# JakeKurtz/MC-Path-Tracer

Hardware: AMD Instinct MI355X
Metric: Mray/s (extend+shade) at 1080p x256spp depth5; fraction of HBM roofline (higher is better)
Workload: dtype f32

## Files before the change

### include/mcpt.h

```cpp
#ifndef MCPT_H
#define MCPT_H
#include <stdint.h>

#ifdef __cplusplus
extern "C" {
#endif

#define MCPT_ABI_VERSION 1

enum {
    MCPT_OK = 0,
    MCPT_E_INVALID = -1,
    MCPT_E_HIP = -2,
    MCPT_E_IO = -3,
    MCPT_E_NOMEM = -4,
    MCPT_E_NODEVICE = -5
};

typedef struct mcpt_config {
    uint64_t seed;
    int32_t spp;
    int32_t max_depth;
    int32_t rr_depth;
    int32_t tile_w;
// ... 32 lines not shown
typedef struct mcpt_camera {
    float inv_view_proj[16];
    float inv_view[16];
    float lens_radius;
    float focal;
} mcpt_camera;

typedef struct mcpt_camera_params {
    float position[3];
    float yaw_deg, pitch_deg;
    float fovy_rad, aspect, znear, zfar;
    float lens_radius, focal;
} mcpt_camera_params;

typedef struct mcpt_stage_stats {
    uint64_t extend_rays;
    uint64_t shadow_rays;
    uint64_t vis_rays;
    uint64_t iterations;
    uint64_t live_paths;
    float ms_total;
    float ms_shade;
    float ms_extend;
    float ms_shadow;
    uint64_t ext_nodes;
    uint64_t ext_tests;
    uint64_t ext_hits;
    uint64_t any_nodes, any_tests, any_hits;
} mcpt_stage_stats;

enum { MCPT_STAGE_LOGIC = 0, MCPT_STAGE_GENERATE = 1, MCPT_STAGE_MATERIAL = 2,
       MCPT_STAGE_EXTEND = 3, MCPT_STAGE_SHADOW = 4 };

typedef struct mcpt_path_view {
    uint32_t film_w, film_h;
    uint32_t *flags, *samples;
    int32_t *hit_tri;
    float *ray_o, *ray_d, *beta, *nee0, *nee1;
    uint8_t *vis;
    float *Ld;
    float *light_o, *light_d, *bvis_o, *bvis_d;
    uint8_t *queued;
} mcpt_path_view;

typedef struct mcpt_soa_view {
    const float *ray_o;
    const float *ray_d;
    float *hit_pos_t;
    float *hit_nrm_mat;
    int32_t *hit_tri;
    uint8_t *visible;
    uint32_t *steps;
    mcpt_path_view *paths;
} mcpt_soa_view;

typedef struct mcpt_ctx mcpt_ctx;
typedef struct mcpt_scene mcpt_scene;

int mcpt_create(int device, const mcpt_config *cfg, mcpt_ctx **out);
void mcpt_destroy(mcpt_ctx *ctx);
const char *mcpt_last_error(const mcpt_ctx *ctx);
int mcpt_scene_upload(mcpt_ctx *ctx, const mcpt_scene_desc *desc);
#define MCPT_GPU_BVH_LBVH 0
#define MCPT_GPU_BVH_PLOC 1
int mcpt_scene_upload_gpu_bvh(mcpt_ctx *ctx, const mcpt_scene_desc *desc);
int mcpt_set_gpu_bvh_builder(mcpt_ctx *ctx, int32_t builder);
#define MCPT_GEOM_REFIT   0
#define MCPT_GEOM_REBUILD 1
int mcpt_scene_update_geometry(mcpt_ctx *ctx, int32_t ntri,
                               const float *v0, const float *v1, const float *v2,
                               const float *n0, const float *n1, const float *n2,
                               int32_t mode);
int mcpt_scene_update_geometry_device(mcpt_ctx *ctx, int32_t ntri, const void *d_v0, const void *d_v1,
                                      const void *d_v2, const void *d_n0, const void *d_n1, const void *d_n2,
                                      int32_t mode);
int mcpt_debug_geometry_update_ms(const mcpt_ctx *ctx, float *out8);
int mcpt_camera_set(mcpt_ctx *ctx, const mcpt_camera *cam);
int mcpt_film_resize(mcpt_ctx *ctx, uint32_t w, uint32_t h, uint32_t tile_w, uint32_t tile_h);
int mcpt_film_clear(mcpt_ctx *ctx);
int mcpt_set_path_slots(mcpt_ctx *ctx, uint32_t slots);
int mcpt_set_trace_partitions(mcpt_ctx *ctx, uint32_t nparts);
int mcpt_set_work_counters(mcpt_ctx *ctx, int32_t on);
int mcpt_set_skip_discarded(mcpt_ctx *ctx, int32_t on);
int mcpt_set_tiles(mcpt_ctx *ctx, const uint32_t *tile_xy, uint32_t ntiles);
int mcpt_set_compact_paths(mcpt_ctx *ctx, int32_t on);
int mcpt_wavefront_step(mcpt_ctx *ctx, uint32_t tile_x, uint32_t tile_y, mcpt_stage_stats *st);
int mcpt_iterate(mcpt_ctx *ctx, uint32_t iterations, mcpt_stage_stats *st);
int mcpt_render(mcpt_ctx *ctx, mcpt_stage_stats *st);
int mcpt_stage_run(mcpt_ctx *ctx, int stage, const mcpt_soa_view *in, mcpt_soa_view *out, uint32_t n);
int mcpt_film_read(mcpt_ctx *ctx, float *Ld_rgb, uint32_t *samples);
int mcpt_film_read_device(mcpt_ctx *ctx, void *d_Ld_rgb, void *d_samples);
int mcpt_film_pack_tiles(mcpt_ctx *ctx, void *d_out, uint32_t *npix);
int mcpt_film_unpack_tiles(mcpt_ctx *ctx, const void *d_in, const uint32_t *tile_xy, uint32_t ntiles);
int mcpt_film_tonemap_rgba8(mcpt_ctx *ctx, float exposure, uint8_t *out);
int mcpt_film_size(const mcpt_ctx *ctx, uint32_t *w, uint32_t *h);
int mcpt_gather(mcpt_ctx *const *ctxs, int32_t n, int32_t root);
int mcpt_film_write_png(mcpt_ctx *ctx, float exposure, const char *path);
int mcpt_film_write_pfm(mcpt_ctx *ctx, const char *path);
int mcpt_image_write_png(const char *path, uint32_t w, uint32_t h, const uint8_t *rgba8);
int mcpt_image_write_pfm(const char *path, uint32_t w, uint32_t h, const float *rgb);
int mcpt_guides_render(mcpt_ctx *ctx, uint32_t nsamples);
int mcpt_guides_read(mcpt_ctx *ctx, float *albedo_rgb, float *normal_xyz, float *depth, uint32_t *count);
typedef struct mcpt_denoise_params {
    int32_t passes;
    float sigma_color;
    float sigma_normal, sigma_albedo, sigma_depth;
} mcpt_denoise_params;
int mcpt_denoise_default_params(mcpt_denoise_params *p);
int mcpt_denoise_run(mcpt_ctx *ctx, uint32_t w, uint32_t h, const float *rgb, const uint32_t *samples,
                     const float *albedo, const float *normal, const float *depth, const mcpt_denoise_params *p,
                     float *out_rgb);
int mcpt_film_denoise(mcpt_ctx *ctx, const mcpt_denoise_params *p);
int mcpt_denoised_read(mcpt_ctx *ctx, float *rgb);
int mcpt_denoised_read_device(mcpt_ctx *ctx, void *d_rgb);
int mcpt_denoised_tonemap_rgba8(mcpt_ctx *ctx, float exposure, uint8_t *out);
int mcpt_denoised_write_png(mcpt_ctx *ctx, float exposure, const char *path);
int mcpt_debug_denoise_ms(const mcpt_ctx *ctx, float *out10);
typedef struct mcpt_denoise_guided_params {
    int32_t passes;
    float sigma_lum;
    float lum_eps;
    float sigma_color;
    float sigma_normal, sigma_albedo, sigma_depth;
} mcpt_denoise_guided_params;
int mcpt_denoise_guided_default_params(mcpt_denoise_guided_params *p);
int mcpt_denoise_guided_run(mcpt_ctx *ctx, uint32_t w, uint32_t h, const float *rgb, const uint32_t *samples,
                            const float *variance, const float *albedo, const float *normal, const float *depth,
                            const mcpt_denoise_guided_params *p, float *out_rgb, float *out_variance);
int mcpt_film_denoise_guided(mcpt_ctx *ctx, const mcpt_denoise_guided_params *p);
int mcpt_denoised_variance_read(mcpt_ctx *ctx, float *var);
int mcpt_set_sample_budget(mcpt_ctx *ctx, const uint32_t *budget);
int mcpt_sample_budget_read(mcpt_ctx *ctx, uint32_t *out);
int mcpt_set_spp(mcpt_ctx *ctx, int32_t spp);
int mcpt_film_error(mcpt_ctx *ctx);
int mcpt_film_error_read(mcpt_ctx *ctx, float *out4);
int mcpt_error_run(mcpt_ctx *ctx, uint32_t w, uint32_t h, uint32_t slots, const float *Ld_slots,
                   const uint32_t *samples_slots, float *out4);
int mcpt_debug_film_read_slot(mcpt_ctx *ctx, uint32_t slot, float *Ld_rgb, uint32_t *samples);
typedef struct mcpt_sample_budget_params {
    float target_rel_err;
    float lum_floor;
    uint32_t min_spp, max_spp;
} mcpt_sample_budget_params;
int mcpt_sample_budget_default_params(mcpt_sample_budget_params *p);
int mcpt_budget_from_error(mcpt_ctx *ctx, const mcpt_sample_budget_params *p, uint64_t *out3);
int64_t mcpt_debug_adaptive_bytes(const mcpt_ctx *ctx);
int mcpt_debug_adaptive_ms(const mcpt_ctx *ctx, float *out2);
int mcpt_set_seed(mcpt_ctx *ctx, uint64_t seed);
int mcpt_camera_view_proj(const mcpt_camera *cam, float *out16);
typedef struct mcpt_temporal_params {
    float pos_tol;
    float nrm_tol;
    float max_history;
    float alpha_min;
} mcpt_temporal_params;
int mcpt_temporal_default_params(mcpt_temporal_params *p);
int mcpt_film_temporal(mcpt_ctx *ctx, const mcpt_temporal_params *p);
int mcpt_temporal_reset(mcpt_ctx *ctx);
int mcpt_temporal_read(mcpt_ctx *ctx, float *rgb, float *nsamples, float *variance, float *position);
int mcpt_temporal_denoise(mcpt_ctx *ctx, const mcpt_denoise_guided_params *p);
int mcpt_temporal_run(mcpt_ctx *ctx, uint32_t w, uint32_t h, const float *rgb, const uint32_t *samples,
                      const float *variance, const float *position, const float *normal, const float *depth,
                      const float *hcol, const float *hpos, const float *hnrm, const float *vp_prev16,
                      const mcpt_temporal_params *p, float *out_col, float *out_vl, float *out_hcol, float *out_hpos,
                      float *out_hnrm);
int64_t mcpt_debug_temporal_bytes(const mcpt_ctx *ctx);
int mcpt_debug_temporal_ms(const mcpt_ctx *ctx, float *out1);
typedef struct mcpt_variance_params {
    int32_t radius;
    float sigma_normal, sigma_albedo, sigma_depth;
    float min_neff;
} mcpt_variance_params;
int mcpt_variance_default_params(mcpt_variance_params *p);
int mcpt_variance_run(mcpt_ctx *ctx, uint32_t w, uint32_t h, const float *rgb, const uint32_t *samples,
                      const float *variance, const float *albedo, const float *normal, const float *depth,
                      const mcpt_variance_params *p, float *out_variance);
int mcpt_set_variance_fill(mcpt_ctx *ctx, const mcpt_variance_params *p);
int mcpt_debug_variance_ms(const mcpt_ctx *ctx, float *out1);
int mcpt_set_material_emission(mcpt_ctx *ctx, int32_t nmat, const float *rgb);
int mcpt_material_emission_read(mcpt_ctx *ctx, float *rgb, int32_t *nmat);
int mcpt_set_emitter_sampling(mcpt_ctx *ctx, int32_t on);
int mcpt_emitter_table_read(mcpt_ctx *ctx, float *cdf, float *pick, uint32_t *tri_id, int32_t *n);
int mcpt_debug_emitter_stats(const mcpt_ctx *ctx, double *out4);
int mcpt_sync(mcpt_ctx *ctx);
int mcpt_device_name(mcpt_ctx *ctx, char *buf, int32_t len);
int mcpt_debug_queue_rays(mcpt_ctx *ctx, int which, float *ray_o, float *ray_d, uint32_t *n_inout);
float mcpt_debug_last_stage_ms(const mcpt_ctx *ctx);
int mcpt_debug_tiny_lds_stack(mcpt_ctx *ctx, int32_t on);
float mcpt_debug_last_build_ms(const mcpt_ctx *ctx);
float mcpt_debug_last_env_build_ms(const mcpt_ctx *ctx);
int mcpt_debug_env_tables(mcpt_ctx *ctx, float *marginal_y, float *conds_y, float *pdf, int32_t *flags);
int mcpt_debug_node_layout(const mcpt_ctx *ctx);
typedef struct mcpt_bvh_info {
    int32_t npairs;
    int32_t root_ref;
    int32_t depth;
    int32_t width;
    int32_t layout;
    int32_t ntri;
    int32_t tri_f4;
    int32_t gpu_built;
    int32_t rounds;
    float root_mn[3], root_mx[3];
    float cull_p;
} mcpt_bvh_info;
int mcpt_debug_bvh_read(mcpt_ctx *ctx, float *nodes, float *tris, mcpt_bvh_info *info);
int mcpt_debug_occ_stats(const mcpt_ctx *ctx, uint64_t *resolved, int32_t *enabled);
int mcpt_debug_occ_complete_stats(const mcpt_ctx *ctx, double *out4);
int mcpt_debug_ray_counts(const mcpt_ctx *ctx, uint64_t *out);
int mcpt_debug_primary_stats(const mcpt_ctx *ctx, double *out4);
int mcpt_debug_discard_stats(const mcpt_ctx *ctx, uint64_t *out4);
int mcpt_debug_trace_profile(mcpt_ctx *ctx, uint64_t *out12, int reset);
int mcpt_debug_shade_sections(mcpt_ctx *ctx, uint64_t *out, int n, int reset);
int mcpt_debug_quot(mcpt_ctx *ctx, const float *a, const float *b, uint32_t n, float *out);
int mcpt_debug_hbm_copy(mcpt_ctx *ctx, uint64_t bytes, uint32_t iters, double *gbps);

mcpt_scene *mcpt_scene_new(void);
void mcpt_scene_free(mcpt_scene *s);
int mcpt_scene_load_glb(mcpt_scene *s, const char *path, const float *xform16);
int mcpt_scene_add_mesh(mcpt_scene *s, int32_t ntri, const float *v0, const float *v1, const float *v2,
                        const float *n0, const float *n1, const float *n2, const float *base_rgb);
int mcpt_scene_set_material_emission(mcpt_scene *s, int32_t mat, const float *rgb);
int mcpt_scene_get_emission(const mcpt_scene *s, const float **rgb, int32_t *nmat);
int mcpt_scene_set_env_hdr(mcpt_scene *s, const char *path, int32_t mode);
#define MCPT_ENV_DEVICE_TABLES 1
int mcpt_scene_set_env_hdr_ex(mcpt_scene *s, const char *path, int32_t mode, uint32_t flags);
int mcpt_scene_set_env_color(mcpt_scene *s, const float *rgb, float ls);
int mcpt_scene_add_dir_light(mcpt_scene *s, const float *dir, const float *rgb, float ls);
int mcpt_scene_transform(mcpt_scene *s, const float *xform16);
int mcpt_scene_make_proxy(mcpt_scene *s, int32_t config_id, const char *asset_dir);
int mcpt_scene_build(mcpt_scene *s, int32_t max_prims_in_node);
#define MCPT_BVH_REFERENCE 0
#define MCPT_BVH_SAH3 1
typedef struct mcpt_bvh_params {
    int32_t builder;
    int32_t max_prims;
    int32_t buckets;
    float trav_cost;
    float isect_cost;
} mcpt_bvh_params;
int mcpt_scene_build_ex(mcpt_scene *s, const mcpt_bvh_params *p);
int mcpt_scene_get_desc(const mcpt_scene *s, mcpt_scene_desc *out);
int mcpt_scene_bvh_depth(const mcpt_scene *s);
int mcpt_camera_make(const mcpt_camera_params *p, mcpt_camera *out);

#ifdef __cplusplus
}
#endif
#endif
```

### include/mcpt.hpp

```cpp
#ifndef MCPT_HPP
#define MCPT_HPP

#include <algorithm>
#include <array>
#include <atomic>
#include <cmath>
#include <cstdint>
#include <cstring>
#include <memory>
#include <stdexcept>
#include <string>
#include <utility>
#include <vector>

#include "mcpt.h"

namespace mcpt {

class Error : public std::runtime_error {
public:
    Error(int code, const std::string& what) : std::runtime_error(what), code_(code) {}
    int code() const { return code_; }

private:
// ... 363 lines not shown
    float get_exposure() const { return exposure; }
    void get_size(uint32_t& w, uint32_t& h) const { w = width; h = height; }
    void get_tile_size(uint32_t& w, uint32_t& h) const { w = tile_width; h = tile_height; }
    uint32_t get_id() const { return id; }
    void clear() {
        tile_id = 0;
        tile_x_pos = 0;
        tile_y_pos = 0;
        ++clears_;
        notify();
    }
    void update_tile_position() {
        tile_id = (tile_id + 1) % nmb_tiles;
        tile_x_pos = tile_id % nmb_tile_cols;
        tile_y_pos = tile_id / nmb_tile_cols;
    }
    uint32_t get_tile_x_pos() const { return tile_x_pos; }
    uint32_t get_tile_y_pos() const { return tile_y_pos; }
    uint32_t get_nmb_tiles() const { return nmb_tiles; }
    const std::vector<uint8_t>& get_image() const { return image; }
    uint64_t clear_count() const { return clears_; }

private:
    friend class PathTracer;
    void update_tile_info() {
        nmb_tile_cols = tile_width ? (width + tile_width - 1) / tile_width : 0;
        nmb_tile_rows = tile_height ? (height + tile_height - 1) / tile_height : 0;
        nmb_tiles = std::max(1u, nmb_tile_cols * nmb_tile_rows);
        nmb_tile_cols = std::max(1u, nmb_tile_cols);
    }
    uint32_t id = detail::gen_id();
    uint32_t width = 1, height = 1, tile_width = 0, tile_height = 0;
    uint32_t tile_id = 0, nmb_tiles = 1, nmb_tile_cols = 1, nmb_tile_rows = 1, tile_x_pos = 0, tile_y_pos = 0;
    float exposure = 1.f;
    uint64_t clears_ = 0;
    std::vector<uint8_t> image;
};

inline mcpt_config default_config() {
    mcpt_config c{0x5EED2026ull, 250, 5, 3, 256, 256, 0};
    return c;
}

class PathTracer {
public:
    explicit PathTracer(int device = 0, mcpt_config cfg = default_config()) : cfg_(cfg) {
        cfg.flags |= MCPT_FLAG_NO_AUTO_CLEAR;
        detail::check(mcpt_create(device, &cfg, &ctx_), nullptr, "PathTracer");
    }
    ~PathTracer() { mcpt_destroy(ctx_); }
    PathTracer(const PathTracer&) = delete;
    PathTracer& operator=(const PathTracer&) = delete;

    const std::vector<uint8_t>& render_image(const std::shared_ptr<Scene>& scene, const std::shared_ptr<Camera>& camera,
                                             const std::shared_ptr<Film>& film) {
        sync(*scene, *camera, *film);
        detail::check(mcpt_wavefront_step(ctx_, film->tile_x_pos, film->tile_y_pos, &stats_), ctx_, "render_image");
        if (display_) tonemap(*film);
        film->update_tile_position();
        return film->image;
    }
    const mcpt_stage_stats& render_iterations(const std::shared_ptr<Scene>& scene, const std::shared_ptr<Camera>& camera,
                                              const std::shared_ptr<Film>& film, uint32_t iterations) {
        sync(*scene, *camera, *film);
        detail::check(mcpt_iterate(ctx_, iterations, &stats_), ctx_, "render_iterations");
        if (display_) tonemap(*film);
        return stats_;
    }
    const mcpt_stage_stats& render_frame(const std::shared_ptr<Scene>& scene, const std::shared_ptr<Camera>& camera,
                                         const std::shared_ptr<Film>& film) {
        sync(*scene, *camera, *film);
        detail::check(mcpt_render(ctx_, &stats_), ctx_, "render_frame");
        if (display_) tonemap(*film);
        return stats_;
    }

    void clear_queues() {}
    void set_samples(int) {}
    int get_samples() { return 0; }

    void set_path_slots(uint32_t slots) {
        detail::check(mcpt_set_path_slots(ctx_, slots), ctx_, "set_path_slots");
    }
    void set_display(bool on) { display_ = on; }
    const mcpt_stage_stats& last_stats() const { return stats_; }
    const mcpt_config& config() const { return cfg_; }
    mcpt_ctx* handle() const { return ctx_; }
    std::string device_name() const {
        char buf[256] = {0};
        detail::check(mcpt_device_name(ctx_, buf, (int32_t)sizeof(buf)), ctx_, "device_name");
        return buf;
    }
    void read_film(std::vector<float>& Ld, std::vector<uint32_t>& samples) {
        uint32_t w = 0, h = 0;
        detail::check(mcpt_film_size(ctx_, &w, &h), ctx_, "read_film");
        Ld.resize((size_t)w * h * 3);
        samples.resize((size_t)w * h);
        detail::check(mcpt_film_read(ctx_, Ld.data(), samples.data()), ctx_, "read_film");
    }
    void write_png(const std::shared_ptr<Film>& film, const std::string& path) {
        detail::check(mcpt_film_write_png(ctx_, film->get_exposure(), path.c_str()), ctx_, "write_png");
    }
    void write_pfm(const std::string& path) {
        detail::check(mcpt_film_write_pfm(ctx_, path.c_str()), ctx_, "write_pfm");
    }
    void denoise(uint32_t guide_samples = 4, const mcpt_denoise_params* params = nullptr) {
        if (guide_samples) detail::check(mcpt_guides_render(ctx_, guide_samples), ctx_, "guides");
        detail::check(mcpt_film_denoise(ctx_, params), ctx_, "denoise");
    }
    void denoise_guided(uint32_t guide_samples = 4, const mcpt_denoise_guided_params* params = nullptr) {
        if (guide_samples) detail::check(mcpt_guides_render(ctx_, guide_samples), ctx_, "guides");
        detail::check(mcpt_film_denoise_guided(ctx_, params), ctx_, "denoise_guided");
    }
    void set_variance_fill(bool on = true, const mcpt_variance_params* params = nullptr) {
        mcpt_variance_params p;
        if (on && !params) detail::check(mcpt_variance_default_params(&p), ctx_, "set_variance_fill");
        detail::check(mcpt_set_variance_fill(ctx_, on ? (params ? params : &p) : nullptr), ctx_, "set_variance_fill");
    }
    void denoised_variance(std::vector<float>& var) {
        uint32_t w = 0, h = 0;
        detail::check(mcpt_film_size(ctx_, &w, &h), ctx_, "denoised_variance");
        var.resize((size_t)w * h);
        detail::check(mcpt_denoised_variance_read(ctx_, var.data()), ctx_, "denoised_variance");
    }
    void denoised(std::vector<float>& rgb) {
        uint32_t w = 0, h = 0;
        detail::check(mcpt_film_size(ctx_, &w, &h), ctx_, "denoised");
        rgb.resize((size_t)w * h * 3);
        detail::check(mcpt_denoised_read(ctx_, rgb.data()), ctx_, "denoised");
    }
    void write_denoised_png(const std::shared_ptr<Film>& film, const std::string& path) {
        detail::check(mcpt_denoised_write_png(ctx_, film->get_exposure(), path.c_str()), ctx_, "write_denoised_png");
    }
    void set_seed(uint64_t seed) {
        detail::check(mcpt_set_seed(ctx_, seed), ctx_, "set_seed");
        cfg_.seed = seed;
    }
    void temporal_accumulate(uint32_t guide_samples = 4, const mcpt_temporal_params* params = nullptr) {
        if (guide_samples) detail::check(mcpt_guides_render(ctx_, guide_samples), ctx_, "guides");
        detail::check(mcpt_film_temporal(ctx_, params), ctx_, "temporal_accumulate");
    }
    void temporal(std::vector<float>& rgb, std::vector<float>& nsamples, std::vector<float>& variance) {
        uint32_t w = 0, h = 0;
        detail::check(mcpt_film_size(ctx_, &w, &h), ctx_, "temporal");
        rgb.resize((size_t)w * h * 3);
        nsamples.resize((size_t)w * h);
        variance.resize((size_t)w * h);
        detail::check(mcpt_temporal_read(ctx_, rgb.data(), nsamples.data(), variance.data(), nullptr), ctx_, "temporal");
    }
    void temporal_denoise(const mcpt_denoise_guided_params* params = nullptr) {
        detail::check(mcpt_temporal_denoise(ctx_, params), ctx_, "temporal_denoise");
    }
    void temporal_reset() { detail::check(mcpt_temporal_reset(ctx_), ctx_, "temporal_reset"); }
    void update_geometry(const std::vector<float>& v0, const std::vector<float>& v1, const std::vector<float>& v2,
                         const std::vector<float>* n0 = nullptr, const std::vector<float>* n1 = nullptr,
                         const std::vector<float>* n2 = nullptr, int32_t mode = MCPT_GEOM_REFIT) {
        if (v0.size() % 3 || v1.size() != v0.size() || v2.size() != v0.size() || (n0 && n0->size() != v0.size()) ||
            (n1 && n1->size() != v0.size()) || (n2 && n2->size() != v0.size()))
            throw Error(MCPT_E_INVALID, "update_geometry: arrays of 3 floats per triangle, all of one size");
        detail::check(mcpt_scene_update_geometry(ctx_, (int32_t)(v0.size() / 3), v0.data(), v1.data(), v2.data(),
                                                 n0 ? n0->data() : nullptr, n1 ? n1->data() : nullptr,
                                                 n2 ? n2->data() : nullptr, mode),
                      ctx_, "update_geometry");
    }
    std::array<float, 8> geometry_update_ms() const {
        std::array<float, 8> ms{};
// ... 138 lines not shown
```

### mc-path-tracer_amd/csrc/kernels.hip

```cpp
#include <hip/hip_runtime.h>
#include <stdint.h>
#include <stdlib.h>
#include <string.h>
#include <algorithm>

#include "device/mcpt_core.hpp"
#include "device/scene_dev.hpp"
#include "kernels.hpp"

using namespace mcpt;

namespace mcpt_dev {

template <int NQ>
__device__ inline void block_push(const bool (&want)[NQ], uint32_t* const (&counters)[NQ], uint32_t (&slot)[NQ],
                                  uint32_t (&total)[NQ]) {
    __shared__ uint32_t s_wave[NQ][kBlock / 64];
    __shared__ uint32_t s_base[NQ];
    __shared__ uint32_t s_tot[NQ];
    const int lane = threadIdx.x & 63, wave = threadIdx.x >> 6;
    uint32_t prefix[NQ];
#pragma unroll
    for (int q = 0; q < NQ; q++) {
        uint64_t m = __ballot(want[q]);
        prefix[q] = __builtin_amdgcn_mbcnt_hi((uint32_t)(m >> 32), __builtin_amdgcn_mbcnt_lo((uint32_t)m, 0u));
        if (lane == 0) s_wave[q][wave] = (uint32_t)__popcll(m);
    }
    __syncthreads();
    if (threadIdx.x < NQ) {
        const int q = threadIdx.x;
        uint32_t tot = 0;
        for (int w = 0; w < kBlock / 64; w++) { uint32_t c = s_wave[q][w]; s_wave[q][w] = tot; tot += c; }
        s_base[q] = tot ? atomicAdd(counters[q], tot) : 0u;
        s_tot[q] = tot;
    }
    __syncthreads();
#pragma unroll
    for (int q = 0; q < NQ; q++) {
        slot[q] = s_base[q] + s_wave[q][wave] + prefix[q];
        total[q] = s_tot[q];
    }
}

template <class T>
__device__ inline const T& kernarg_fresh() {
    typedef const __attribute__((address_space(4))) T KT;
    KT* p = (KT*)__builtin_amdgcn_kernarg_segment_ptr();
    __asm__ volatile("" : "+s"(p));
    return *(const T*)p;
}


#ifndef MCPT_NT
#define MCPT_NT 3
#endif
template <class T>
__device__ inline void st_q(T* p, T v) {
    if constexpr (MCPT_NT & 8) __builtin_nontemporal_store(v, p);
    else *p = v;
}
typedef float f4v_t __attribute__((ext_vector_type(4)));
typedef uint32_t u4v_t __attribute__((ext_vector_type(4)));
template <class T>
__device__ inline T ld_s(const T* p) {
    if constexpr (MCPT_NT & 1) return __builtin_nontemporal_load(p);
    else return *p;
}
__device__ inline float4 ld_s(const float4* p) {
    if constexpr (MCPT_NT & 1) {
        const f4v_t v = __builtin_nontemporal_load(reinterpret_cast<const f4v_t*>(p));
        return make_float4(v.x, v.y, v.z, v.w);
    } else {
        return *p;
    }
}
__device__ inline uint4 ld_s(const uint4* p) {
    if constexpr (MCPT_NT & 1) {
        const u4v_t v = __builtin_nontemporal_load(reinterpret_cast<const u4v_t*>(p));
        return make_uint4(v.x, v.y, v.z, v.w);
    } else {
        return *p;
    }
}
template <class T>
__device__ inline void st_s(T* p, T v) {
    if constexpr (MCPT_NT & 2) __builtin_nontemporal_store(v, p);
    else *p = v;
}
// ... 1 lines not shown
    if constexpr (MCPT_NT & 2) __builtin_nontemporal_store(f4v_t{v.x, v.y, v.z, v.w}, reinterpret_cast<f4v_t*>(p));
    else *p = v;
}
__device__ inline void st_s(uint4* p, uint4 v) {
    if constexpr (MCPT_NT & 2) __builtin_nontemporal_store(u4v_t{v.x, v.y, v.z, v.w}, reinterpret_cast<u4v_t*>(p));
    else *p = v;
}

enum : int { SD_WAVES = 0, SD_VALID, SD_LOGIC, SD_NEE, SD_GEN, SD_CONT, SD_BG, SD_N };
#ifdef MCPT_DIAG_SHADE
__device__ unsigned long long g_shade_diag[2 * SD_N];
#define SHADE_DIAG(k, cond)                                                      \
    do {                                                                         \
        const uint64_t m_ = __ballot(cond);                                      \
        if ((threadIdx.x & 63) == 0 && m_) {                                     \
            atomicAdd(&g_shade_diag[2 * (k)], 1ull);                             \
            atomicAdd(&g_shade_diag[2 * (k) + 1], (unsigned long long)__popcll(m_)); \
        }                                                                        \
    } while (0)
#else
#define SHADE_DIAG(k, cond) \
    do {                    \
    } while (0)
#endif
int shade_sections(unsigned long long* out, int n, int reset) {
#ifdef MCPT_DIAG_SHADE
    unsigned long long h[2 * SD_N];
    if (hipMemcpyFromSymbol(h, HIP_SYMBOL(g_shade_diag), sizeof(h)) != hipSuccess) return -1;
    for (int i = 0; i < n && i < 2 * SD_N; i++) out[i] = h[i];
    if (reset) {
        memset(h, 0, sizeof(h));
        if (hipMemcpyToSymbol(HIP_SYMBOL(g_shade_diag), h, sizeof(h)) != hipSuccess) return -1;
    }
    return 2 * SD_N;
#else
    for (int i = 0; i < n; i++) out[i] = 0;
    (void)reset;
    return 0;
#endif
}

__device__ inline V3 light_L(const DevScene& sc, int id, V3 wi) {
    if (id == 0) return env_L(sc.env, wi);
    const float* p = sc.dirs + 7 * (id - 1);
    return v3(p[3], p[4], p[5]) * p[6];
}
template <bool FIXED>
__device__ inline void light_L_pdf(const DevScene& sc, int id, V3 wi, V3& L, float& pdf) {
    if (id == 0) {
        env_L_pdf<FIXED>(sc.env, wi, L, pdf);
    } else {
        const float* p = sc.dirs + 7 * (id - 1);
        L = v3(p[3], p[4], p[5]) * p[6];
        pdf = 1.f;
    }
}
__device__ inline float light_pdf(const DevScene& sc, int id, V3 wi) {
    if (id == 0) return env_pdf(sc.env, wi);
    return 1.f;
}

__device__ inline bool slab(float mnx, float mny, float mnz, float mxx, float mxy, float mxz, V3 o, V3 inv,
                            int nx, int ny, int nz, float& t0, float& t1) {
    float bx0 = nx ? mxx : mnx, bx1 = nx ? mnx : mxx;
    float by0 = ny ? mxy : mny, by1 = ny ? mny : mxy;
    float bz0 = nz ? mxz : mnz, bz1 = nz ? mnz : mxz;
    float tmin = (bx0 - o.x) * inv.x;
    float tmax = (bx1 - o.x) * inv.x;
    float tymin = (by0 - o.y) * inv.y;
    float tymax = (by1 - o.y) * inv.y;
    float tzmin = (bz0 - o.z) * inv.z;
    float tzmax = (bz1 - o.z) * inv.z;
    bool miss = (tmin > tymax) || (tymin > tmax);
    float a = (tymin > tmin) ? tymin : tmin;
    float b = (tymax < tmax) ? tymax : tmax;
    miss = miss || (a > tzmax) || (tzmin > b);
    t0 = (tzmin > a) ? tzmin : a;
    t1 = (tzmax < b) ? tzmax : b;
    return !miss;
}
constexpr float K_INF_F = __builtin_huge_valf();

__device__ inline float cull_iota(const DevScene& sc, V3 d, V3 inv) {
    const float ax = __builtin_fabsf(inv.x), ay = __builtin_fabsf(inv.y), az = __builtin_fabsf(inv.z);
    if (!(ax < K_INF_F && ay < K_INF_F && az < K_INF_F)) return -K_INF_F;
    const float n2 = d.x * d.x + d.y * d.y + d.z * d.z;
    if (!sc.cull_ok || !(n2 <= kCullNormMax)) return -3.4028235e38f;
    const float io = __builtin_fmaxf(__builtin_fmaxf(ax, ay), az) * kCullSlackF;
    return io * sc.cull_p <= 1.f ? io : -io;
}
__device__ inline bool keep_box(float t0, float t1, float m, float cut, float& key) {
    key = t0 - __builtin_fabsf(m);
    return !(m >= 0.f && __builtin_fmaf(t1, kCullBehindF, m) < 0.f) && !(key > cut);
}

typedef float f2v __attribute__((ext_vector_type(2)));
__device__ inline void pair_slab(float4 qx, float4 qy, float4 qz, V3 o, V3 inv, float& t0a, float& t1a, float& t0b,
                                 float& t1b) {
    const f2v ox = {o.x, o.x}, oy = {o.y, o.y}, oz = {o.z, o.z};
    const f2v ix = {inv.x, inv.x}, iy = {inv.y, inv.y}, iz = {inv.z, inv.z};
    const f2v ax = (f2v{qx.x, qx.y} - ox) * ix, bx = (f2v{qx.z, qx.w} - ox) * ix;
    const f2v ay = (f2v{qy.x, qy.y} - oy) * iy, by = (f2v{qy.z, qy.w} - oy) * iy;
    const f2v az = (f2v{qz.x, qz.y} - oz) * iz, bz = (f2v{qz.z, qz.w} - oz) * iz;
    t0a = __builtin_fmaxf(__builtin_fmaxf(__builtin_fminf(ax.x, bx.x), __builtin_fminf(ay.x, by.x)),
                          __builtin_fminf(az.x, bz.x));
    t1a = __builtin_fminf(__builtin_fminf(__builtin_fmaxf(ax.x, bx.x), __builtin_fmaxf(ay.x, by.x)),
                          __builtin_fmaxf(az.x, bz.x));
    t0b = __builtin_fmaxf(__builtin_fmaxf(__builtin_fminf(ax.y, bx.y), __builtin_fminf(ay.y, by.y)),
                          __builtin_fminf(az.y, bz.y));
    t1b = __builtin_fminf(__builtin_fminf(__builtin_fmaxf(ax.y, bx.y), __builtin_fmaxf(ay.y, by.y)),
                          __builtin_fmaxf(az.y, bz.y));
}

__device__ inline void quad_axis(const float4& mn, const float4& mx, float o, float inv, float (&lo)[4],
                                 float (&hi)[4], bool first) {
    const f2v oo = {o, o}, ii = {inv, inv};
    const f2v a0 = (f2v{mn.x, mn.y} - oo) * ii, a1 = (f2v{mn.z, mn.w} - oo) * ii;
    const f2v b0 = (f2v{mx.x, mx.y} - oo) * ii, b1 = (f2v{mx.z, mx.w} - oo) * ii;
    const float l[4] = {__builtin_fminf(a0.x, b0.x), __builtin_fminf(a0.y, b0.y), __builtin_fminf(a1.x, b1.x),
                        __builtin_fminf(a1.y, b1.y)};
    const float h[4] = {__builtin_fmaxf(a0.x, b0.x), __builtin_fmaxf(a0.y, b0.y), __builtin_fmaxf(a1.x, b1.x),
                        __builtin_fmaxf(a1.y, b1.y)};
#pragma unroll
    for (int k = 0; k < 4; k++) {
        lo[k] = first ? l[k] : __builtin_fmaxf(lo[k], l[k]);
        hi[k] = first ? h[k] : __builtin_fminf(hi[k], h[k]);
    }
}

__device__ inline f2v pk_slab(f2v q, f2v p) {
    f2v r;
    __asm__("v_pk_add_f32 %0, %1, %2 op_sel_hi:[1,0] neg_lo:[0,1] neg_hi:[0,1]\n\t"
            "v_pk_mul_f32 %0, %0, %2 op_sel:[0,1] op_sel_hi:[1,1]"
            : "=&v"(r)
            : "v"(q), "v"(p));
    return r;
}
__device__ inline void box_t(float ax, float bx, float ay, float by, float az, float bz, float& t0, float& t1) {
    float m0, m1, m2, n0, n1, n2;
    __asm__("v_min_f32 %2, %8, %9\n\t"
            "v_min_f32 %3, %10, %11\n\t"
            "v_min_f32 %4, %12, %13\n\t"
            "v_max_f32 %5, %8, %9\n\t"
            "v_max_f32 %6, %10, %11\n\t"
            "v_max_f32 %7, %12, %13\n\t"
            "v_max3_f32 %0, %2, %3, %4\n\t"
            "v_min3_f32 %1, %5, %6, %7"
            : "=v"(t0), "=v"(t1), "=&v"(m0), "=&v"(m1), "=&v"(m2), "=&v"(n0), "=&v"(n1), "=&v"(n2)
            : "v"(ax), "v"(bx), "v"(ay), "v"(by), "v"(az), "v"(bz));
}
__device__ inline void pair_slab2(float4 qx, float4 qy, float4 qz, f2v px, f2v py, f2v pz, float& t0a, float& t1a,
                                  float& t0b, float& t1b) {
    const f2v ax = pk_slab(f2v{qx.x, qx.y}, px), bx = pk_slab(f2v{qx.z, qx.w}, px);
    const f2v ay = pk_slab(f2v{qy.x, qy.y}, py), by = pk_slab(f2v{qy.z, qy.w}, py);
    const f2v az = pk_slab(f2v{qz.x, qz.y}, pz), bz = pk_slab(f2v{qz.z, qz.w}, pz);
    box_t(ax.x, bx.x, ay.x, by.x, az.x, bz.x, t0a, t1a);
    box_t(ax.y, bx.y, ay.y, by.y, az.y, bz.y, t0b, t1b);
}
__device__ inline float vmin(float a, float b) {
    float r;
    __asm__("v_min_f32 %0, %1, %2" : "=v"(r) : "v"(a), "v"(b));
    return r;
}
__device__ inline float vmax(float a, float b) {
    float r;
    __asm__("v_max_f32 %0, %1, %2" : "=v"(r) : "v"(a), "v"(b));
    return r;
}
__device__ inline void quad_axis2(const float4& mn, const float4& mx, f2v p, float (&lo)[4], float (&hi)[4], bool first) {
    const f2v a0 = pk_slab(f2v{mn.x, mn.y}, p), a1 = pk_slab(f2v{mn.z, mn.w}, p);
    const f2v b0 = pk_slab(f2v{mx.x, mx.y}, p), b1 = pk_slab(f2v{mx.z, mx.w}, p);
    const float l[4] = {vmin(a0.x, b0.x), vmin(a0.y, b0.y), vmin(a1.x, b1.x), vmin(a1.y, b1.y)};
    const float h[4] = {vmax(a0.x, b0.x), vmax(a0.y, b0.y), vmax(a1.x, b1.x), vmax(a1.y, b1.y)};
#pragma unroll
    for (int k = 0; k < 4; k++) {
        lo[k] = first ? l[k] : vmax(lo[k], l[k]);
        hi[k] = first ? h[k] : vmin(hi[k], h[k]);
    }
}

__device__ inline bool ray_misses_scene(const DevScene& sc, V3 o, V3 d) {
    if (!(d.x == d.x && d.y == d.y && d.z == d.z) || (d.x == 0.f && d.y == 0.f && d.z == 0.f)) return true;
    if (o.x >= sc.root_mn[0] && o.x <= sc.root_mx[0] && o.y >= sc.root_mn[1] && o.y <= sc.root_mx[1] &&
        o.z >= sc.root_mn[2] && o.z <= sc.root_mx[2])
        return false;
    const V3 inv = v3(1.f / d.x, 1.f / d.y, 1.f / d.z);
    const float m = sc.root_w * cull_iota(sc, d, inv);
    float t0, t1, key;
    return !(slab(sc.root_mn[0], sc.root_mn[1], sc.root_mn[2], sc.root_mx[0], sc.root_mx[1], sc.root_mx[2], o, inv,
                  inv.x < 0.f, inv.y < 0.f, inv.z < 0.f, t0, t1) &&
             keep_box(t0, t1, m, K_INF_F, key));
}

__device__ inline bool occ_test(V3 o, V3 d, V3 inv, float io, float4 bmn, float4 bmx, float4 r2, float4 r3) {
    const float ax = (bmn.x - o.x) * inv.x, bx = (bmx.x - o.x) * inv.x;
    const float ay = (bmn.y - o.y) * inv.y, by = (bmx.y - o.y) * inv.y;
    const float az = (bmn.z - o.z) * inv.z, bz = (bmx.z - o.z) * inv.z;
    const float t0 = __builtin_fmaxf(__builtin_fmaxf(__builtin_fminf(ax, bx), __builtin_fminf(ay, by)),
                                     __builtin_fminf(az, bz));
    const float t1 = __builtin_fminf(__builtin_fminf(__builtin_fmaxf(ax, bx), __builtin_fmaxf(ay, by)),
                                     __builtin_fmaxf(az, bz));
    float key;
    if (!(t0 <= t1) || !keep_box(t0, t1, bmn.w * io, K_INF_F, key)) return false;
    float th;
    return tri_test_t(o, d, v3(bmx.w, r2.x, r2.y), v3(r2.z, r2.w, r3.x), v3(r3.y, r3.z, r3.w), th) && !(th < 0.f) &&
           th < K_HUGE;
}
struct OccEnt { uint32_t w[kOccWays]; };
__device__ inline OccEnt occ_entry(const DevScene& sc, uint32_t cell) {
    typedef uint32_t uwv_t __attribute__((ext_vector_type(kOccWays)));
    const uwv_t* e = reinterpret_cast<const uwv_t*>(sc.occ) + cell;
    uwv_t v;
    if constexpr (MCPT_NT & 16) v = __builtin_nontemporal_load(e);
    else v = *e;
    OccEnt r;
#pragma unroll
    for (uint32_t k = 0; k < kOccWays; k++) r.w[k] = v[k];
    return r;
}
enum : int { kOccOpen = 0, kOccHit = 1, kOccMaybe = 2 };
__device__ inline int occ_hit1(const DevScene& sc, V3 o, V3 d, OccEnt e, bool& done) {
    done = sc.occ_dir != nullptr;
    bool any = false;
#pragma unroll
    for (uint32_t k = 0; k < kOccWays; k++) done = done && mcpt::occ_word_done(e.w[k]);
#pragma unroll
    for (uint32_t k = 0; k < kOccWays; k++) {
        if (done) e.w[k] &= mcpt::kOccDoneIndex;
        any = any || e.w[k] < sc.ntri;
    }
    if (!(any || done)) return kOccOpen;
    const V3 inv = v3(1.f / d.x, 1.f / d.y, 1.f / d.z);
    const bool fin = __builtin_fabsf(inv.x) < K_INF_F && __builtin_fabsf(inv.y) < K_INF_F && __builtin_fabsf(inv.z) < K_INF_F;
    const float io = cull_iota(sc, d, inv);
#pragma unroll
    for (uint32_t k = 0; k < kOccWays; k += 2) {
        const bool v0 = e.w[k] < sc.ntri, v1 = e.w[k + 1] < sc.ntri;
        if (kOccWays > 2 && !(v0 || v1)) continue;
        const float4* p0 = sc.occ_rec + kOccRecF4 * (size_t)(v0 ? e.w[k] : 0u);
        const float4* p1 = sc.occ_rec + kOccRecF4 * (size_t)(v1 ? e.w[k + 1] : 0u);
        const float4 bn0 = p0[0], bx0 = p0[1], r20 = p0[2], r30 = p0[3];
        const float4 bn1 = p1[0], bx1 = p1[1], r21 = p1[2], r31 = p1[3];
        if (!fin) return kOccOpen;
        if ((v0 && occ_test(o, d, inv, io, bn0, bx0, r20, r30)) || (v1 && occ_test(o, d, inv, io, bn1, bx1, r21, r31)))
            return kOccHit;
    }
    return done && fin && io > 0.f ? kOccMaybe : kOccOpen;
}
__device__ inline void occ_member2(const DevScene& sc, V3 ol, V3 dl, uint32_t kl, V3 ob, V3 db, uint32_t kb, bool& m_l,
                                   bool& m_b) {
    const mcpt::OccGrid g{{sc.root_mn[0], sc.root_mn[1], sc.root_mn[2]}, {sc.occ_cell[0], sc.occ_cell[1], sc.occ_cell[2]},
                          sc.occ_g, sc.occ_b, sc.occ_dir};
    const mcpt::Beam bl = mcpt::occ_key_beam(g, (kl >> 15) & 31u, (kl >> 20) & 31u, kl >> 25, kl & 0x7fffu);
    const mcpt::Beam bb = mcpt::occ_key_beam(g, (kb >> 15) & 31u, (kb >> 20) & 31u, kb >> 25, kb & 0x7fffu);
    m_l = mcpt::beam_contains(bl, ol, dl);
    m_b = mcpt::beam_contains(bb, ob, db);
}

struct MatOut {
    bool want_ext, want_l, want_b, trivial_ext, vis_ray, need_cb;
    bool skip_ext;
    bool doomed_inplace;
    uint32_t trivial_any;
    OccEnt el, eb;
    uint32_t kl, kb;
    V3 n, wo, wi_b;
    int matid, light_id;
    uint32_t flags;
    float rrz;
};

template <bool FIXED, bool SAMP = false>
__device__ inline MatOut material(const ShadeArgs& a, uint32_t pid, uint32_t pix, uint32_t sidx, uint32_t len,
                                 V3 beta_store, int32_t htri, float4* stage, bool occ_on, bool no_cont, bool& want_e) {
    const DevScene& sc = a.scene;
    MatOut mo{};
#pragma unroll
    for (uint32_t k = 0; k < kOccWays; k++) mo.el.w[k] = mo.eb.w[k] = kOccEmpty;
    MCPT_MARK("m_hit");
    const Rng r{rng_key(a.seed, pix, sidx), len};
    const V3 ro = xyz(ld_s(a.p.ray_o + pid)), rdir = xyz(ld_s(a.p.ray_d + pid));
    V3 pos, n;
    int mat;
    float t_hit;
    hit_record(sc, ro, rdir, htri, pos, n, mat, t_hit);
    const V3 wo = -rdir;
    const Mat m = load_mat(sc.mats + 8 * mat);
    uint32_t nf = 0;
    V3 rr;
    if (no_cont) {
        rr = v3(0.f, 0.f, 0.f);
        st_s(a.p.beta + pid, f4(beta_store, 0.f));
        mo.skip_ext = true;
    } else {
        MCPT_MARK("m_cont");
        V3 wi_s = brdf_sample_wi<FIXED>(m, n, wo, r, SL_CONT_E0, r(SL_CONT_LOBE) < 0.5f);
        float pdf_s;
        V3 f_s;
        brdf_f_pdf(m, n, wi_s, wo, f_s, pdf_s);
        if ((f_s.x == 0.f && f_s.y == 0.f && f_s.z == 0.f) || pdf_s == 0.f) nf |= F_FZERO;
        rr = f_s / pdf_s;
        const V3 new_o = pos + n * 0.001f;
        st_s(a.p.beta + pid, f4(beta_store, rr.x));
        bool doomed = false;
        if (FIXED || !a.skip) {
            doomed = len + 1u > (uint32_t)a.max_depth;
            if (!doomed && len + 1u > (uint32_t)a.rr_depth) {
                const Rng r1{r.key, len + 1u};
                float q;
                doomed = rr_terminates(r1, FIXED ? (beta_store * rr).y : beta_store.y, q);
            }
        }
        if (doomed && a.skip) {
            mo.skip_ext = true;
        } else {
            st_s(a.p.ray_o + pid, f4(new_o, 0.f));
            st_s(a.p.ray_d + pid, f4(wi_s, 0.f));
            mo.want_ext = true;
            if (ray_misses_scene(sc, new_o, wi_s)) {
                a.p.hit_tri[pid] = -1;
                mo.want_ext = false;
                mo.trivial_ext = true;
                mo.doomed_inplace = doomed;
            }
        }
    }
    MCPT_MARK("m_light");
    int l_id = (int)(r(SL_LIGHT) * (float)(sc.nlights - 0) + (float)0);
    const int light_id = (l_id == sc.nlights) ? 0 : l_id;
    const bool delta = light_id > 0;
    const float sel = FIXED ? 1.f / (float)sc.nlights : 1.f;
    {
        V3 ldir, Li_l;
        float pdfl_x;
        const float4* lt = sc.env.ltab[FIXED ? 1 : 0];
        if (light_id == 0 && lt) {
            int cx, cy;
            env_cell<FIXED>(sc.env, r, cx, cy);
            const float4 t0 = lt[(int64_t)cy * (sc.env.w + 1) + cx + 1];
            const float2 rs = sc.env.lrow[FIXED ? 1 : 0][cy], cs = sc.env.lcol[FIXED ? 1 : 0][cx + 1];
            ldir = v3(cs.y * rs.x, rs.y, cs.x * rs.x);
            pdfl_x = t0.w;
            Li_l = xyz(t0);
        } else {
            if (light_id == 0) ldir = env_dir<FIXED>(sc.env, r);
            else ldir = ld3(sc.dirs + 7 * (light_id - 1), 0);
            light_L_pdf<FIXED>(sc, light_id, ldir, Li_l, pdfl_x);
        }
        V3 f_l;
        float pdf_bl;
        brdf_f_pdf(m, n, ldir, wo, f_l, pdf_bl);
        if (FIXED) pdfl_x = pdfl_x * sel;
        float pdfb_y = !delta ? pdf_bl : (FIXED ? 0.f : 1.f);
        float wL = power_heuristic(pdfl_x, pdfb_y);
        V3 cL = ((f_l * Li_l) * wL) / pdfl_x;
        if (wL > 0.f && pdfl_x > 0.f) nf |= F_CONDL;
        st_s(a.p.nee0 + pid, f4(cL, rr.y));
        const V3 so_l = pos + n * 0.01f;
        if (ray_misses_scene(sc, so_l, ldir)) {
            a.p.vis[2 * pid] = 1;
            mo.trivial_any++;
        } else {
            stage[0 * kBlock + threadIdx.x] = f4(so_l, __uint_as_float(2 * pid));
            stage[1 * kBlock + threadIdx.x] = f4(ldir, 0.f);
            mo.want_l = true;
            if (occ_on) mo.el = occ_entry(sc, occ_index(sc, so_l, ldir, &mo.kl));
        }
    }
    if constexpr (SAMP) {
        MCPT_MARK("m_emit");
        int k = upper_bound(a.emit_cdf, a.emit_n, r(SL_EMIT_PICK));
        k = k < a.emit_n - 1 ? k : a.emit_n - 1;
        const uint2 ent = a.emit_ent[k];
        const float4* tp = sc.tri + (size_t)kTriF4 * ent.x;
        const float4 w0 = tp[0], w1 = tp[1], w2 = tp[2];
        const V3 ev0 = v3(w0.x, w0.y, w0.z), e1 = v3(w0.w, w1.x, w1.y), e2 = v3(w1.z, w1.w, w2.x);
        const float u1 = r(SL_EMIT_U), u2 = r(SL_EMIT_V), su = __builtin_sqrtf(u1);
        const V3 pe = (ev0 + e1 * (su * (1.f - u2))) + e2 * (su * u2);
        const V3 so_e = pos + n * 0.01f;
        const V3 dv = pe - so_e;
        const float d2 = dot(dv, dv), dist = __builtin_sqrtf(d2);
        const V3 edir = dv / dist;
        const V3 c = cross(e1, e2);
        const float area = 0.5f * __builtin_sqrtf(dot(c, c));
        const float cosl = __builtin_fabsf(dot(normalize(c), edir));
        const float pdf_e = ((__uint_as_float(ent.y) / area) * d2) / cosl;
        V3 f_e;
        float pdf_be;
        brdf_f_pdf(m, n, edir, wo, f_e, pdf_be);
        const int mat_e = __float_as_int(sc.tri_sh[3 * (size_t)ent.x + 2].y);
        V3 cE = (f_e * ld3f4(a.emis + mat_e)) / pdf_e;
        const bool ok = dist > 0.f && cosl > 0.f && pdf_e > 0.f && pdf_e < K_INF_F && __builtin_fabsf(cE.x) < K_INF_F &&
                        __builtin_fabsf(cE.y) < K_INF_F && __builtin_fabsf(cE.z) < K_INF_F;
        if (ok) {
            stage[4 * kBlock + threadIdx.x] = f4(so_e, __uint_as_float(a.emit_vis0 + pid));
            stage[5 * kBlock + threadIdx.x] = f4(edir, dist * 0.999f);
            want_e = true;
        } else {
            cE = v3(0.f, 0.f, 0.f);
            a.p.vis[a.emit_vis0 + pid] = 0;
        }
        st_s(a.nee2 + pid, f4(cE, 0.f));
    }
    MCPT_MARK("m_bsdir");
    if (!delta) {
        const V3 wi_b = brdf_sample_wi<FIXED>(m, n, wo, r, SL_MAT_E0, r(SL_MAT_LOBE) < 0.5f);
// ... 294 lines not shown
            const uint32_t qi = shard * a.ext_cap + slot[1];
            st_s(a.mat_rec + qi, make_uint4(pid, pix, cont_sidx | (no_cont ? kRecNoCont : 0u) | (cont_len << kRecLenShift),
                                            (uint32_t)cont_htri));
            st_s(a.mat_beta + qi, f4(beta_store, 0.f));
        }
    }
    uint32_t n_ext = ((gen_ext || gen_trivial || gen_prim) ? 1u : 0u) + (dd ? 1u : 0u);
    for (int off = 32; off > 0; off >>= 1) n_ext += __shfl_xor(n_ext, off);
    if (lane == 0 && n_ext) atomicAdd(sc_ctr + C_EXT_RAYS, n_ext);
    if (a.skip) {
        const uint32_t n_dd = (uint32_t)__popcll(__ballot(dd)), n_ddv = (uint32_t)__popcll(__ballot(dd_vis));
        if (lane == 0 && n_dd) {
            atomicAdd(sc_ctr + C_ANY_RAYS, n_dd + n_ddv);
            if (n_ddv) atomicAdd(sc_ctr + C_VIS, n_ddv);
            atomicAdd(sc_ctr + C_SKIP_EXT, n_dd);
            atomicAdd(sc_ctr + C_SKIP_ANY, n_dd + n_ddv);
            atomicAdd(sc_ctr + C_SKIP_MAT, n_dd);
        }
    }
    if (a.prim_cnt) {
        const uint32_t n_prim = (uint32_t)__popcll(__ballot(prim_res));
        if (lane == 0 && n_prim) atomicAdd(sc_ctr + C_PRIM_RAYS, n_prim);
    }
    MCPT_MARK("background");
    if (bg) {
        const int nbg = FIXED ? 1 : sc.nlights;
        V3 film = bg_film;
        for (int i = 0; i < nbg; i++) film = film + env_L(sc.env, bg_dir) * v3(1.f, 1.f, 1.f);
        if (__float_as_uint(film.x) != __float_as_uint(bg_film.x) || __float_as_uint(film.y) != __float_as_uint(bg_film.y) ||
            __float_as_uint(film.z) != __float_as_uint(bg_film.z))
            a.p.Ld[pid] = f4(film, 0.f);
    }
    if constexpr (EMIT) {
        MCPT_MARK("emission");
        if (em) {
            const int mat = __float_as_int(sc.tri_sh[3 * cont_htri + 2].y);
            const V3 film = bg_film + ld3f4(a.emis + mat) * beta_store;
            if (em_dirty || __float_as_uint(film.x) != __float_as_uint(bg_film.x) ||
                __float_as_uint(film.y) != __float_as_uint(bg_film.y) || __float_as_uint(film.z) != __float_as_uint(bg_film.z))
                a.p.Ld[pid] = f4(film, 0.f);
        }
    }
    MCPT_MARK("done");
    if (a.blk_done && __syncthreads_and(finished ? 1 : 0) && threadIdx.x == 0) a.blk_done[v.done] = 1;
    MCPT_MARK("end");
}

template <bool FIXED, bool MAP, bool EMIT, bool SAMP = false>
__global__ __launch_bounds__(kBlock) MCPT_SHADE_ATTR void k_shade(ShadeArgs a) {
    if (a.cnt->idle) return;
    __shared__ uint64_t s_live[kBlock / 64];
    const uint32_t G = gridDim.x, nvb = a.shade_vblocks;
    const uint32_t mine = (nvb - blockIdx.x + G - 1) / G;
    const uint32_t k = threadIdx.x;
    bool live = false;
    __shared__ VBlk s_vb[kBlock];
    if (k < mine) {
        const VBlk v = vblock_of(a, (int)(blockIdx.x + k * G));
        live = !a.blk_done || a.blk_done[v.done] == 0;
        s_vb[k] = v;
    }
    const uint64_t m = __ballot(live);
    if ((threadIdx.x & 63) == 0) s_live[threadIdx.x >> 6] = m;
    __syncthreads();
    for (uint32_t j = 0; j < mine; j++) {
        if (!((s_live[j >> 6] >> (j & 63)) & 1ull)) continue;
        shade_vblock<FIXED, MAP, EMIT, SAMP>(kernarg_fresh<ShadeArgs>(), (int)(blockIdx.x + j * G), s_vb[j]);
    }
}

template <bool FIXED, bool SAMP = false>
__global__ __launch_bounds__(kBlock) MCPT_MAT_ATTR void k_material(ShadeArgs a_kernarg) {
    (void)a_kernarg;
    const ShadeArgs& a = kernarg_fresh<ShadeArgs>();
    if (a.cnt->idle) return;
    const uint32_t shard = blockIdx.x % kShards, w_in = blockIdx.x / kShards, bps = gridDim.x / kShards;
    uint32_t* sc_ctr = a.cnt->shard[shard];
    const uint32_t n = sc_ctr[C_MAT];
    const int lane = threadIdx.x & 63;
    uint32_t n_ext = 0, n_any = 0, n_vis = 0, n_occ = 0, occ_try = 0, n_skip = 0, n_inpl = 0, n_dvis = 0, n_docc = 0;
    uint32_t n_emit = 0;
    (void)n_emit;
    const bool occ_on = a.scene.occ && a.scene.occ_gate[0] == 0 && a.scene.occ_gate[2] != 0;
    __shared__ float4 s_any[SAMP ? 6 : 4][kBlock];
    for (uint32_t base = w_in * kBlock; base < n; base += bps * kBlock) {
        const ShadeArgs& a = kernarg_fresh<ShadeArgs>();
        const uint32_t i = base + threadIdx.x;
        MatOut mo{};
        bool want_e = false;
        uint32_t mpid = 0;
        bool occ_l = false, occ_b = false, try_l = false, try_b = false;
        bool done_l = false, done_b = false, clr_l = false, clr_b = false;
        if (i < n) {
            const uint4 q = ld_s(a.mat_rec + shard * a.ext_cap + i);
            const float4 b4 = ld_s(a.mat_beta + shard * a.ext_cap + i);
            mpid = q.x;
            mo = material<FIXED, SAMP>(a, mpid, q.y, q.z & (kRecNoCont - 1u), q.z >> kRecLenShift, xyz(b4), (int32_t)q.w,
                                 &s_any[0][0], occ_on, (q.z & kRecNoCont) != 0u, want_e);
            MCPT_MARK("m_occ");
            if (occ_on) {
                try_l = mo.want_l;
                try_b = mo.want_b;
                const V3 ol = xyz(s_any[0][threadIdx.x]), dl = xyz(s_any[1][threadIdx.x]);
                const V3 ob = xyz(s_any[2][threadIdx.x]), db = xyz(s_any[3][threadIdx.x]);
                if (mo.want_l) {
                    const int r = occ_hit1(a.scene, ol, dl, mo.el, done_l);
                    occ_l = r == kOccHit;
                    clr_l = r == kOccMaybe;
                }
                if (mo.want_b) {
                    const int r = occ_hit1(a.scene, ob, db, mo.eb, done_b);
                    occ_b = r == kOccHit;
                    clr_b = r == kOccMaybe;
                }
                if (clr_l || clr_b) {
                    bool m_l, m_b;
                    occ_member2(a.scene, ol, dl, mo.kl, ob, db, mo.kb, m_l, m_b);
                    clr_l = clr_l && m_l;
                    clr_b = clr_b && m_b;
                }
                if (clr_l) {
                    a.p.vis[2 * mpid] = 1;
                    mo.want_l = false;
                    mo.trivial_any++;
                }
                if (clr_b) {
                    a.p.vis[2 * mpid + 1] = 1;
                    mo.want_b = false;
                    mo.trivial_any++;
                }
                if (occ_l) {
                    a.p.vis[2 * mpid] = 0;
                    mo.want_l = false;
                    mo.trivial_any++;
                }
                if (occ_b) {
                    a.p.vis[2 * mpid + 1] = 0;
                    mo.want_b = false;
                    mo.need_cb = false;
                    mo.trivial_any++;
                }
            }
            MCPT_MARK("m_bterms");
            material_brdf_terms<FIXED>(a, mpid, mo);
        }
        MCPT_MARK("m_push");
        uint32_t slot[SAMP ? 4 : 3], total[SAMP ? 4 : 3];
        if constexpr (SAMP) {
            bool want[4] = {mo.want_ext, mo.want_l, mo.want_b, want_e};
            uint32_t* ctr[4] = {sc_ctr + C_EXT, sc_ctr + C_ANY, sc_ctr + C_ANY, sc_ctr + C_ANY};
            block_push<4>(want, ctr, slot, total);
        } else {
            bool want[3] = {mo.want_ext, mo.want_l, mo.want_b};
            uint32_t* ctr[3] = {sc_ctr + C_EXT, sc_ctr + C_ANY, sc_ctr + C_ANY};
            block_push<3>(want, ctr, slot, total);
        }
        if (mo.want_ext) st_q(a.ext_q + shard * a.ext_cap + slot[0], mpid);
        if (mo.want_l) {
            const uint32_t k = shard * a.any_cap + slot[1];
            if constexpr (MCPT_NT & 8) {
                st_s(a.p.sray_o + k, s_any[0][threadIdx.x]);
                st_s(a.p.sray_d + k, s_any[1][threadIdx.x]);
            } else {
                a.p.sray_o[k] = s_any[0][threadIdx.x];
                a.p.sray_d[k] = s_any[1][threadIdx.x];
            }
        }
        if (mo.want_b) {
            const uint32_t k = shard * a.any_cap + slot[2];
            if constexpr (MCPT_NT & 8) {
                st_s(a.p.sray_o + k, s_any[2][threadIdx.x]);
                st_s(a.p.sray_d + k, s_any[3][threadIdx.x]);
            } else {
                a.p.sray_o[k] = s_any[2][threadIdx.x];
                a.p.sray_d[k] = s_any[3][threadIdx.x];
            }
        }
        if constexpr (SAMP) {
            if (want_e) {
                const uint32_t k = shard * a.any_cap + slot[3];
                if constexpr (MCPT_NT & 8) {
                    st_s(a.p.sray_o + k, s_any[4][threadIdx.x]);
                    st_s(a.p.sray_d + k, s_any[5][threadIdx.x]);
                } else {
                    a.p.sray_o[k] = s_any[4][threadIdx.x];
                    a.p.sray_d[k] = s_any[5][threadIdx.x];
                }
            }
            n_emit += (uint32_t)__popcll(__ballot(want_e));
        }
        MCPT_MARK("m_count");
        n_occ += (uint32_t)(__popcll(__ballot(occ_l)) + __popcll(__ballot(occ_b)));
        occ_try += (uint32_t)(__popcll(__ballot(try_l)) + __popcll(__ballot(try_b)));
        n_dvis += (uint32_t)(__popcll(__ballot(clr_l)) + __popcll(__ballot(clr_b)));
        n_docc += (uint32_t)(__popcll(__ballot(occ_l && done_l)) + __popcll(__ballot(occ_b && done_b)));
        n_ext += (uint32_t)__popcll(__ballot(mo.want_ext || mo.trivial_ext || mo.skip_ext));
        n_skip += (uint32_t)__popcll(__ballot(mo.skip_ext));
        n_inpl += (uint32_t)__popcll(__ballot(mo.doomed_inplace));
        n_any += (uint32_t)(__popcll(__ballot(mo.want_l)) + __popcll(__ballot(mo.want_b)) +
                            __popcll(__ballot(mo.trivial_any >= 1u)) + __popcll(__ballot(mo.trivial_any >= 2u)));
        n_vis += (uint32_t)__popcll(__ballot(mo.vis_ray));
    }
    if (lane == 0) {
        if (n_ext) atomicAdd(sc_ctr + C_EXT_RAYS, n_ext);
        if (n_any) atomicAdd(sc_ctr + C_ANY_RAYS, n_any);
        if (n_vis) atomicAdd(sc_ctr + C_VIS, n_vis);
        if (n_occ) atomicAdd(sc_ctr + C_OCC, n_occ);
        if (occ_try) atomicAdd(sc_ctr + C_OCC_TRY, occ_try);
        if (n_dvis) atomicAdd(sc_ctr + C_OCC_DONE_VIS, n_dvis);
        if (n_docc) atomicAdd(sc_ctr + C_OCC_DONE_OCC, n_docc);
        if (n_skip) atomicAdd(sc_ctr + C_SKIP_EXT, n_skip);
        if (n_inpl) atomicAdd(sc_ctr + C_SKIP_INPLACE, n_inpl);
        if constexpr (SAMP)
            if (n_emit) atomicAdd(a.cnt->tot_emit + shard, (unsigned long long)n_emit);
    }
}

__device__ inline uint32_t wave_scan_incl(uint32_t x) {
    x += (uint32_t)__builtin_amdgcn_update_dpp(0, (int)x, 0x111, 0xf, 0xf, false);
    x += (uint32_t)__builtin_amdgcn_update_dpp(0, (int)x, 0x112, 0xf, 0xf, false);
    x += (uint32_t)__builtin_amdgcn_update_dpp(0, (int)x, 0x114, 0xf, 0xf, false);
    x += (uint32_t)__builtin_amdgcn_update_dpp(0, (int)x, 0x118, 0xf, 0xf, false);
    x += (uint32_t)__builtin_amdgcn_update_dpp(0, (int)x, 0x142, 0xa, 0xf, false);
    x += (uint32_t)__builtin_amdgcn_update_dpp(0, (int)x, 0x143, 0xc, 0xf, false);
    return x;
}

__device__ inline void wave_stats(uint32_t* stats, int lane, uint32_t nodes, uint32_t tests, uint32_t hits) {
    if (!stats) return;
    for (int off = 32; off > 0; off >>= 1) {
        nodes += __shfl_xor(nodes, off);
        tests += __shfl_xor(tests, off);
        hits += __shfl_xor(hits, off);
    }
    if (lane == 0) {
        uint32_t* st = stats + (blockIdx.x % kShards) * C_WORDS;
        atomicAdd(st + 0, nodes);
        atomicAdd(st + 1, tests);
        atomicAdd(st + 2, hits);
    }
}

#ifndef MCPT_NODE_STEPS
#define MCPT_NODE_STEPS 4
#endif
#ifndef MCPT_TRI_SHARE
#define MCPT_TRI_SHARE 0
#endif
constexpr int kShareMaxStack = 8;
constexpr int kNodeSteps = MCPT_NODE_STEPS;
#ifndef MCPT_GRAB_MAX
#define MCPT_GRAB_MAX 0
#endif
constexpr int kGrabMax = MCPT_GRAB_MAX;
#ifndef MCPT_ANY_FIRST
#define MCPT_ANY_FIRST 0
#endif
constexpr bool kAnyFirst = MCPT_ANY_FIRST != 0;
#ifndef MCPT_NODE_MIN_LANES2
#define MCPT_NODE_MIN_LANES2 32
#endif
#ifndef MCPT_NODE_MIN_LANES2_DEEP
#define MCPT_NODE_MIN_LANES2_DEEP 0
#endif
#ifndef MCPT_NODE_MIN_LANES4
#define MCPT_NODE_MIN_LANES4 24
#endif

#ifndef MCPT_TRACE_WPE
#define MCPT_TRACE_WPE 7
#endif
#ifndef MCPT_TRACE_WPE_DEEP
#define MCPT_TRACE_WPE_DEEP 7
#endif
#ifndef MCPT_TRACE_WPE4
#define MCPT_TRACE_WPE4 6
#endif
#define MCPT_TRACE_WPE_OF(kW, kS) \
    ((kW) == 4 ? MCPT_TRACE_WPE4 : ((kS) > ::mcpt_dev::kLdsStack ? MCPT_TRACE_WPE_DEEP : MCPT_TRACE_WPE))
#define MCPT_TRACE_ATTR \
    __attribute__((amdgpu_waves_per_eu(MCPT_TRACE_WPE_OF(kW, kLdsStack), MCPT_TRACE_WPE_OF(kW, kLdsStack))))
template <int kW, int kLdsStack, bool kCount>
__global__ __launch_bounds__(kTraceBlock) MCPT_TRACE_ATTR void k_trace(TraceArgs a) {
    if (a.idle && *a.idle) return;
    constexpr bool kShare = MCPT_TRI_SHARE != 0 && kLdsStack <= kShareMaxStack;
    __shared__ int2 stk[kLdsStack][kTraceBlock];
    __shared__ uint64_t s_key[kShare ? kTraceBlock : 1];
    const int lane = threadIdx.x;
    const uint32_t nsh = (uint32_t)a.nshards, nparts = a.nparts;
    uint32_t home = 0;
    if (nparts > 1) {
        uint32_t xcc;
        __asm__ volatile("s_getreg_b32 %0, hwreg(HW_REG_XCC_ID)" : "=s"(xcc));
        const uint32_t nd = a.ndies >= 1 && a.ndies <= nparts && nparts % a.ndies == 0 ? a.ndies : nparts;
        home = (xcc & 15u) % nd + nd * ((blockIdx.x / nd) % (nparts / nd));
// ... 418 lines not shown
                float t;
                bool done = false;
                const bool acc = tri_test_t(RAY_O, d, v3(w0.x, w0.y, w0.z), v3(w0.w, w1.x, w1.y), v3(w1.z, w1.w, w2.x), t);
                MCPT_MARK("t_tri2");
                if (acc && !(t < 0.f) &&
                    (best < 0.f ? t < -best
                          : (t < best ||
                             (t == best && tri >= 0 && __float_as_int(w2.y) < __float_as_int(sc.tri[kTriF4 * tri + 2].y))))) {
                    if (best < 0.f) {
                        tri = id;
                        done = true;
                    } else {
                        best = t;
                        tri = id;
                        cut = best * __builtin_fmaf(__builtin_fabsf(io), sc.cull_p, kCullSlackF);
                    }
                }
                if (done) {
                    leaf = kEnd;
                    ref = kEnd;
                } else if ((leaf & 0x07000000) != 0) {
                    leaf = leaf + 1 - (1 << 24);
                } else {
                    leaf = kEnd;
                }
            }
        }
        MCPT_MARK("t_finish");
        if constexpr (kCount) ph[PH_FINISH_TRIPS] += __ballot(act && ref == kEnd && leaf == kEnd) != 0 ? 1u : 0u;
        if (act && ref == kEnd && leaf == kEnd) finish();
        }
        MCPT_MARK("t_end");
    }
    MCPT_MARK("t_scan");
    {
        uint32_t g = 0;
        const bool cand = (uint32_t)lane < nparts && !((drained >> lane) & 1ull);
        if (cand) g = __hip_atomic_load(a.grab + lane * C_WORDS, __ATOMIC_RELAXED, __HIP_MEMORY_SCOPE_AGENT);
        const uint64_t open = __ballot(cand && g < s_tot[lane]);
        if (open == 0) break;
        const uint32_t rem = min(s_tot[lane] - g, (1u << 25) - 1u);
        uint32_t key = (open >> lane) & 1ull ? (rem << 6) | (63u - (uint32_t)lane) : 0u;
        for (int off = 32; off > 0; off >>= 1) key = max(key, (uint32_t)__shfl_xor((int)key, off));
        enter(63u - (__builtin_amdgcn_readfirstlane(key) & 63u));
    }
    }
#undef RAY_O
#undef RAY_INV
    if constexpr (kCount) {
        wave_stats(a.set[0].stats, lane, tot_n - tot_n1, tot_t - tot_t1, tot_h - tot_h1);
        wave_stats(a.set[1].stats, lane, tot_n1, tot_t1, tot_h1);
        if (a.phase && lane == 0) {
            uint32_t* pw = a.phase + (blockIdx.x % kShards) * C_WORDS;
#pragma unroll
            for (int k = 0; k < kPhaseWords; k++)
                if (ph[k]) atomicAdd(pw + k, ph[k]);
        }
    }
}

__global__ __launch_bounds__(kBlock) void k_primary(ShadeArgs a_kernarg) {
    (void)a_kernarg;
    const ShadeArgs& a = kernarg_fresh<ShadeArgs>();
    if (a.cnt->idle) return;
    const uint32_t shard = blockIdx.x % kShards, w_in = blockIdx.x / kShards, bps = gridDim.x / kShards;
    const uint32_t n = a.cnt->shard[shard][C_PRIM];
    const float4* rec = a.scene.occ_rec;
    for (uint32_t i = w_in * kBlock + threadIdx.x; i < n; i += bps * kBlock) {
        const uint2 q = a.prim_q[shard * a.ext_cap + i];
        const V3 o = ld3f4(a.p.ray_o + q.x), d = ld3f4(a.p.ray_d + q.x);
        const uint32_t nc = (uint32_t)a.prim_cnt[q.y] - 1u;
        const uint4* lp = reinterpret_cast<const uint4*>(a.prim_list + (size_t)kPrimLine * q.y);
        const V3 inv = v3(1.f / d.x, 1.f / d.y, 1.f / d.z);
        float best = K_HUGE;
        int32_t tri = -1;
        for (uint32_t j0 = 0; j0 < nc; j0 += 4) {
            const uint4 ids = lp[j0 >> 2];
            const uint32_t id4[4] = {ids.x, ids.y, ids.z, ids.w};
#pragma unroll
            for (int k = 0; k < 4; k++) {
                if (j0 + k >= nc) break;
                const float4* p = rec + kOccRecF4 * (size_t)id4[k];
                const float4 bmn = p[0], bmx = p[1], r2 = p[2], r3 = p[3];
                const float ax = (bmn.x - o.x) * inv.x, bx = (bmx.x - o.x) * inv.x;
                const float ay = (bmn.y - o.y) * inv.y, by = (bmx.y - o.y) * inv.y;
                const float az = (bmn.z - o.z) * inv.z, bz = (bmx.z - o.z) * inv.z;
                const float t0 = __builtin_fmaxf(__builtin_fmaxf(__builtin_fminf(ax, bx), __builtin_fminf(ay, by)),
                                                 __builtin_fminf(az, bz));
                const float t1 = __builtin_fminf(__builtin_fminf(__builtin_fmaxf(ax, bx), __builtin_fmaxf(ay, by)),
                                                 __builtin_fmaxf(az, bz));
                float t;
                if (t0 <= t1 && tri_test_t(o, d, v3(bmx.w, r2.x, r2.y), v3(r2.z, r2.w, r3.x), v3(r3.y, r3.z, r3.w), t) &&
                    !(t < 0.f) && t < best) {
                    best = t;
                    tri = (int32_t)id4[k];
                }
            }
        }
        a.p.hit_tri[q.x] = tri;
    }
}
void launch_primary(const ShadeArgs& a, const LaunchGeom& g, hipStream_t s) {
    if (a.prim_cnt) hipLaunchKernelGGL(k_primary, dim3(g.prim_blocks), dim3(kBlock), 0, s, a);
}

#ifndef MCPT_OCC_BACKOFF0
#define MCPT_OCC_BACKOFF0 15
#endif
__global__ void k_accumulate(CounterBlock* c, uint32_t nparts, uint32_t* occ_gate) {
    if (c->idle) return;
    const int t = threadIdx.x;
    uint32_t v[C_STATS + 6];
#pragma unroll
    for (int k = 0; k < C_STATS + 6; k++) {
        v[k] = c->shard[t][k];
        c->shard[t][k] = 0;
    }
    c->last_ext_shard[t] = v[C_EXT];
    __shared__ uint32_t s_part[kMaxParts];
    if (t < kMaxParts) s_part[t] = 0;
    __syncthreads();
    atomicAdd(&s_part[t % nparts], v[C_EXT] + v[C_ANY]);
    __syncthreads();
    uint32_t g = 0;
    if (t < kMaxParts) g = c->grab[t][0];
    const bool short_part = t < (int)nparts && g < s_part[t];
#pragma unroll
    for (int k = 0; k < C_STATS + 6; k++)
        for (int off = 32; off > 0; off >>= 1) v[k] += __shfl_xor(v[k], off);
    if (__ballot(short_part) != 0 && t == 0) c->trace_short += 1;
    if (t < kMaxParts) c->grab[t][0] = 0;
    uint32_t phw[kPhaseWords];
#pragma unroll
    for (int k = 0; k < kPhaseWords; k++) {
        phw[k] = c->shard[t][C_PH + k];
        c->shard[t][C_PH + k] = 0;
        for (int off = 32; off > 0; off >>= 1) phw[k] += __shfl_xor(phw[k], off);
    }
    uint32_t er = c->shard[t][C_EXT_RAYS], ar = c->shard[t][C_ANY_RAYS], oc = c->shard[t][C_OCC],
             ot = c->shard[t][C_OCC_TRY], pr = c->shard[t][C_PRIM_RAYS], dv = c->shard[t][C_OCC_DONE_VIS],
             dc = c->shard[t][C_OCC_DONE_OCC];
    const int skw[4] = {C_SKIP_EXT, C_SKIP_ANY, C_SKIP_MAT, C_SKIP_INPLACE};
    uint32_t sk[4];
#pragma unroll
    for (int k = 0; k < 4; k++) {
        sk[k] = c->shard[t][skw[k]];
        if (sk[k]) c->shard[t][skw[k]] = 0;
        for (int off = 32; off > 0; off >>= 1) sk[k] += __shfl_xor(sk[k], off);
    }
    c->shard[t][C_PRIM] = 0;
    c->shard[t][C_PRIM_RAYS] = 0;
    c->shard[t][C_EXT_RAYS] = 0;
    c->shard[t][C_ANY_RAYS] = 0;
    c->shard[t][C_MAT] = 0;
    c->shard[t][C_OCC] = 0;
    c->shard[t][C_OCC_TRY] = 0;
    if (dv) c->shard[t][C_OCC_DONE_VIS] = 0;
    if (dc) c->shard[t][C_OCC_DONE_OCC] = 0;
    for (int off = 32; off > 0; off >>= 1) {
        dv += __shfl_xor(dv, off);
        dc += __shfl_xor(dc, off);
        er += __shfl_xor(er, off);
        ar += __shfl_xor(ar, off);
        oc += __shfl_xor(oc, off);
        ot += __shfl_xor(ot, off);
        pr += __shfl_xor(pr, off);
    }
    if (t == 0) {
        c->tot_ext += er;
        c->tot_prim += pr;
        for (int k = 0; k < 4; k++) c->tot_skip[k] += sk[k];
        c->tot_any += ar;
        c->tot_occ += oc;
        c->tot_done[0] += dv;
        c->tot_done[1] += dc;
        if (occ_gate) {
            if (occ_gate[0]) {
                occ_gate[0]--;
            } else if (!occ_gate[2]) {
                if (v[C_ANY]) occ_gate[2] = 1;
            } else if (ot >= 4096u) {
                if (((unsigned long long)oc + dv) * kOccMinRate < ot) {
                    occ_gate[1] = occ_gate[1] ? min(2u * occ_gate[1] + 1u, 255u) : (uint32_t)MCPT_OCC_BACKOFF0;
                    occ_gate[0] = occ_gate[1];
                } else {
                    occ_gate[1] = 0;
                }
            }
        }
        c->tot_vis += v[C_VIS];
        c->tot_ext_q += v[C_EXT];
        c->tot_any_q += v[C_ANY];
        c->last_ext = v[C_EXT];
        c->last_live = er;
        if (er == 0) c->idle = 1;
        for (int k = 0; k < 6; k++) c->tot_stats[k] += v[C_STATS + k];
        for (int k = 0; k < kPhaseWords; k++) c->tot_phase[k] += phw[k];
    }
}
void launch_accumulate(CounterBlock* c, uint32_t nparts, uint32_t* occ_gate, hipStream_t s) {
    hipLaunchKernelGGL(k_accumulate, dim3(1), dim3(kShards), 0, s, c, std::min<uint32_t>(kMaxParts, std::max<uint32_t>(1, nparts)),
                       occ_gate);
}

static uint32_t env_u32(const char* name, int def, int lo, int hi) {
    const char* e = getenv(name);
    int v = e ? atoi(e) : def;
    return (uint32_t)std::min(hi, std::max(lo, v));
}
int launch_geometry(int dev, LaunchGeom& g) {
    int cus = 0, nx = 1, per_cu = 0, mat0 = 0, mat1 = 0, sh0 = 0;
    if (hipDeviceGetAttribute(&cus, hipDeviceAttributeMultiprocessorCount, dev) != hipSuccess) return -1;
    if (hipDeviceGetAttribute(&nx, hipDeviceAttributeNumberOfXccs, dev) != hipSuccess) nx = 1;
    int occ[2][2] = {};
    if (hipOccupancyMaxActiveBlocksPerMultiprocessor(&occ[0][0], k_trace<2, kLdsStack, false>, kTraceBlock, 0) != hipSuccess ||
        hipOccupancyMaxActiveBlocksPerMultiprocessor(&occ[0][1], k_trace<2, kLdsStackDeep, false>, kTraceBlock, 0) != hipSuccess ||
        hipOccupancyMaxActiveBlocksPerMultiprocessor(&occ[1][0], k_trace<4, kLdsStack, false>, kTraceBlock, 0) != hipSuccess ||
        hipOccupancyMaxActiveBlocksPerMultiprocessor(&occ[1][1], k_trace<4, kLdsStackDeep, false>, kTraceBlock, 0) != hipSuccess ||
        hipOccupancyMaxActiveBlocksPerMultiprocessor(&mat0, k_material<false>, kBlock, 0) != hipSuccess ||
        hipOccupancyMaxActiveBlocksPerMultiprocessor(&mat1, k_material<true>, kBlock, 0) != hipSuccess ||
        hipOccupancyMaxActiveBlocksPerMultiprocessor(&sh0, k_shade<false, false, false>, kBlock, 0) != hipSuccess)
        return -1;
    if (cus <= 0) cus = 256;
    per_cu = 32;
    if (const char* e = getenv("MCPT_TRACE_WAVES")) per_cu = atoi(e);
    if (per_cu <= 0) per_cu = 16;
    for (int w = 0; w < 2; w++)
        for (int k = 0; k < 2; k++) g.trace_waves[w][k] = (uint32_t)(cus * std::max(1, std::min(per_cu, occ[w][k])));
    g.ndies = (uint32_t)std::max(1, nx);
    g.trace_parts = env_u32("MCPT_TRACE_PARTS", std::min(kMaxParts, 2 * std::max(1, nx)), 1, kMaxParts);
    if (const char* e = getenv("MCPT_MAT_BLOCKS_PER_CU")) {
        const int m = atoi(e);
        if (m > 0) { mat0 = std::min(mat0, m); mat1 = std::min(mat1, m); }
    }
    g.mat_blocks[0] = (uint32_t)std::max(1, cus * std::max(1, mat0) / kShards) * (uint32_t)kShards;
    g.mat_blocks[1] = (uint32_t)std::max(1, cus * std::max(1, mat1) / kShards) * (uint32_t)kShards;
    {
        int ms0 = 0, ms1 = 0;
        if (hipOccupancyMaxActiveBlocksPerMultiprocessor(&ms0, k_material<false, true>, kBlock, 0) != hipSuccess ||
            hipOccupancyMaxActiveBlocksPerMultiprocessor(&ms1, k_material<true, true>, kBlock, 0) != hipSuccess)
            return -1;
        g.mat_blocks_samp[0] = (uint32_t)std::max(1, cus * std::max(1, ms0) / kShards) * (uint32_t)kShards;
        g.mat_blocks_samp[1] = (uint32_t)std::max(1, cus * std::max(1, ms1) / kShards) * (uint32_t)kShards;
    }
    int prim = 0;
    if (hipOccupancyMaxActiveBlocksPerMultiprocessor(&prim, k_primary, kBlock, 0) != hipSuccess) return -1;
    g.prim_blocks = (uint32_t)std::max(1, cus * std::max(1, prim) / kShards) * (uint32_t)kShards;
    g.shade_grid = (uint32_t)std::max(1, cus * std::max(1, sh0)) * env_u32("MCPT_SHADE_GRID", 16, 0, 1024);
    if (getenv("MCPT_SHADE_WGS")) g.shade_grid = env_u32("MCPT_SHADE_WGS", 0, 1, 1 << 30);
    g.refill_min = env_u32("MCPT_REFILL_MIN", 0, 0, 64);
    g.tri_min = env_u32("MCPT_TRI_MIN", 16, 0, 64);
    return 0;
}
static uint32_t shade_grid(uint32_t nblocks, const LaunchGeom& g) {
    uint32_t G = g.shade_grid ? std::min(nblocks, g.shade_grid) : nblocks;
    return std::max(G, (nblocks + kBlock - 1) / kBlock);
}
void launch_shade(const ShadeArgs& args, int nblocks, const LaunchGeom& g, bool fixed_mode, hipStream_t s) {
    ShadeArgs a = args;
    a.shade_vblocks = (uint32_t)nblocks;
    const uint32_t G = shade_grid((uint32_t)nblocks, g);
    if (a.nee2 && a.emis) {
        if (fixed_mode) {
            if (a.budget) hipLaunchKernelGGL((k_shade<true, true, true, true>), dim3(G), dim3(kBlock), 0, s, a);
            else hipLaunchKernelGGL((k_shade<true, false, true, true>), dim3(G), dim3(kBlock), 0, s, a);
            hipLaunchKernelGGL((k_material<true, true>), dim3(g.mat_blocks_samp[1]), dim3(kBlock), 0, s, a);
        } else {
            if (a.budget) hipLaunchKernelGGL((k_shade<false, true, true, true>), dim3(G), dim3(kBlock), 0, s, a);
            else hipLaunchKernelGGL((k_shade<false, false, true, true>), dim3(G), dim3(kBlock), 0, s, a);
            hipLaunchKernelGGL((k_material<false, true>), dim3(g.mat_blocks_samp[0]), dim3(kBlock), 0, s, a);
        }
        return;
    }
    if (fixed_mode) {
// ... 63 lines not shown
```

### mc-path-tracer_amd/csrc/kernels.hpp

```cpp
#pragma once
#include <hip/hip_runtime.h>
#include <stdint.h>

#include "device/adaptive.hpp"
#include "device/denoise.hpp"
#include "device/mcpt_core.hpp"
#include "device/occ_beam.hpp"
#include "device/temporal.hpp"
#include "device/variance.hpp"

namespace mcpt_dev {

constexpr int kBlock = 256;
constexpr int kTraceBlock = 64;
#ifndef MCPT_LDS_STACK
#define MCPT_LDS_STACK 8
#endif
constexpr int kLdsStack = MCPT_LDS_STACK;
#ifndef MCPT_LDS_STACK_DEEP
#define MCPT_LDS_STACK_DEEP 10
#endif
constexpr int kLdsStackDeep = MCPT_LDS_STACK_DEEP;
constexpr int kLdsStackTiny = 2;
#ifndef MCPT_DEEP_TREE
#define MCPT_DEEP_TREE 20
#endif
constexpr int kDeepTree = MCPT_DEEP_TREE;
constexpr int kMaxStack = 64;

enum : uint32_t {
    F_DEAD = 1u,
    F_LEN_SHIFT = 1,
    F_CONDL = 1u << 9,
    F_CONDB = 1u << 10,
    F_FZERO = 1u << 11,
    F_HASVIS = 1u << 12,
    F_SIDX_SHIFT = 13
};
constexpr uint32_t kMaxSpp = 1u << (32 - F_SIDX_SHIFT);
constexpr int kRecLenShift = 24;
static_assert(kMaxSpp <= (1u << kRecLenShift), "sample index and len share a record word");
constexpr uint32_t kRecNoCont = 1u << 23;
static_assert(kMaxSpp <= kRecNoCont && kRecNoCont < (1u << kRecLenShift), "the mark lies between sample index and len");

__host__ __device__ constexpr int shade_blocks_per_tile(int tile_px, int slots) {
    return (tile_px + kBlock - 1) / kBlock * slots;
}

#ifndef MCPT_TRI_F4
#define MCPT_TRI_F4 3
#endif
constexpr int kTriF4 = MCPT_TRI_F4;

struct DevScene {
    const float4* nodes;
    const float4* tri;
    const float4* tri_sh;
    float root_mn[3], root_mx[3];
    int root_ref;
    int depth;
    int width;
    int nlights;
    const float* mats;
    const float* dirs;
    mcpt::EnvView env;
    uint32_t* occ;
    uint32_t* occ_gate;
    const float4* occ_rec;
    uint32_t ntri;
    int occ_g, occ_b;
    float occ_inv[3];
    const float4* occ_dir;
    float occ_cell[3];
    float cull_p, root_w;
    int cull_ok;
};
constexpr char kOccCompleteEnv[] = "MCPT_OCC_COMPLETE";
constexpr uint32_t kOccEmpty = 0xffffffffu;
#ifndef MCPT_OCC_WAYS
#define MCPT_OCC_WAYS 2
#endif
constexpr uint32_t kOccWays = MCPT_OCC_WAYS;
static_assert(kOccWays == 2 || kOccWays == 4, "an entry is one 8-B or 16-B load");
constexpr uint32_t kOccGateWords = 3;
constexpr uint32_t kOccMinRate = 10;
__host__ __device__ constexpr size_t occ_entries(int g, int b) { return (size_t)g * g * g * 6 * b * b * kOccWays; }

struct DevPaths {
    float4 *ray_o, *ray_d, *sray_o, *sray_d, *beta, *nee0, *nee1, *Ld;
    int32_t* hit_tri;
    uint32_t *flags, *samples;
    uint8_t* vis;
};

constexpr int kShards = 64;
constexpr int kMaxParts = kShards;
enum : int { C_EXT = 0, C_ANY = 1, C_VIS = 2, C_STATS = 3, C_EXT_RAYS = 9, C_ANY_RAYS = 10, C_MAT = 11, C_OCC = 12,
              C_OCC_TRY = 13, C_PH = 14, C_SKIP_INPLACE = 25, C_PRIM = 26, C_PRIM_RAYS = 27, C_SKIP_EXT = 28,
              C_SKIP_ANY = 29, C_SKIP_MAT = 30, C_OCC_DONE_VIS = 31, C_OCC_DONE_OCC = 32, C_WORDS = 64 };
enum : int {
    PH_TRIPS = 0,
    PH_REFILLS = 1,
    PH_REFILL_LANES = 2,
    PH_NODE_ITERS = 3,
    PH_TRI_PHASES = 4,
    PH_TRI_LANES = 5,
    PH_TRIP_NODE = 6,
    PH_TRIP_LEAF = 7,
    PH_TRIP_IDLE = 8,
    PH_FINISH_TRIPS = 9,
    PH_POP_ITERS = 10,
    kPhaseWords = 11
};
struct CounterBlock {
    uint32_t shard[kShards][C_WORDS];
    uint32_t last_ext, last_live;
    uint32_t trace_short;
    uint32_t idle;
    uint32_t pad[28];
    uint32_t last_ext_shard[kShards];
    uint32_t grab[kMaxParts][C_WORDS];
    unsigned long long tot_ext, tot_any, tot_vis, tot_occ;
    unsigned long long tot_stats[6];
    unsigned long long tot_ext_q, tot_any_q;
    unsigned long long tot_phase[kPhaseWords];
    unsigned long long tot_prim;
    unsigned long long tot_skip[4];
    unsigned long long tot_done[2];
    unsigned long long tot_emit[kShards];
};
static_assert(C_PH + kPhaseWords <= C_SKIP_INPLACE, "counter words overlap");

constexpr char kPrimaryHitsEnv[] = "MCPT_PRIMARY_HITS";
constexpr int kPrimLine = 16;
constexpr int kPrimK = kPrimLine;

struct ShadeArgs {
    DevScene scene;
    mcpt::CamView cam;
    DevPaths p;
    const int2* tiles;
    int ntiles, tile_w, tile_h, W, H;
    int spp, max_depth, rr_depth;
    int slots;
    float slots_rcp;
    uint32_t npx;
    int compact;
    const int* tile_base;
    uint64_t seed;
    uint32_t *ext_q, *any_q;
    uint4* mat_rec;
    float4* mat_beta;
    uint32_t ext_cap, any_cap;
    CounterBlock* cnt;
    uint8_t* blk_done;
    uint32_t shade_vblocks;
    const float4* cam_px;
    const float4* cam_dir;
    const uint8_t* prim_cnt;
    const uint32_t* prim_list;
    uint2* prim_q;
    int skip;
    const uint32_t* budget;
    const float4* emis;
    const float* emit_cdf;
    const uint2* emit_ent;
    int emit_n;
    uint32_t emit_vis0;
    float4* nee2;
};
struct PrimaryBuildArgs {
    DevScene scene;
    mcpt::CamView cam;
    int W, H;
    const float4 *cam_px, *cam_dir;
    uint8_t* cnt;
    uint32_t* list;
    uint32_t* stats;
};

struct TraceSet {
    const float4 *ro, *rd;
    const uint32_t* queue;
    const uint32_t* count_ptr;
    uint32_t count;
    uint32_t shard_cap;
    uint32_t* stats;
    uint32_t* ray_steps;
    int prefiltered;
    int ray_at_slot;
};
struct TraceArgs {
    DevScene scene;
    TraceSet set[2];
    int nshards;
    int32_t* hit_tri;
    uint8_t* vis;
    uint32_t refill_min;
    uint32_t tri_min;
    uint32_t nparts;
    uint32_t ndies;
    uint32_t* grab;
    const uint32_t* idle;
    int tiny_stack;
    uint32_t* phase;
};

struct HitRecordArgs { DevScene scene; const float4 *ro, *rd; const int32_t* tri; float4 *hit_p, *hit_n; int32_t* scene_tri; uint32_t n; };
struct ClearArgs { uint32_t* flags; uint32_t* samples; float4* Ld; uint32_t n, npx; };
struct ResolveArgs {
    const float4* Ld; const uint32_t* samples; float4* out_Ld; uint32_t* out_samples; uint32_t n; int slots;
    const int2* tiles; int tile_w, tile_h, W, H;
};
struct TonemapArgs { const float4* Ld; const uint32_t* samples; uchar4* out; float exposure; uint32_t n; };
struct PackArgs { const float4* Ld; const uint32_t* samples; const int2* tiles; int ntiles, tile_w, tile_h, W, H; float4* out; };
struct UnpackArgs { const float4* in; const int2* tiles; int ntiles, tile_w, tile_h, W, H; float4* Ld; uint32_t* samples; };

struct LaunchGeom {
    uint32_t trace_waves[2][2];
    uint32_t trace_parts;
    uint32_t ndies;
    uint32_t mat_blocks[2];
    uint32_t mat_blocks_samp[2];
    uint32_t prim_blocks;
    uint32_t shade_grid;
    uint32_t refill_min, tri_min;
};

int launch_geometry(int device, LaunchGeom& g);
void launch_shade(const ShadeArgs& a, int nblocks, const LaunchGeom& g, bool fixed_mode, hipStream_t s);
void launch_shade_stage(bool material_stage, const ShadeArgs& a, int nblocks, const LaunchGeom& g, bool fixed_mode,
                        hipStream_t s);
void launch_primary(const ShadeArgs& a, const LaunchGeom& g, hipStream_t s);
void launch_trace(const TraceArgs& a, const LaunchGeom& g, hipStream_t s);
void launch_accumulate(CounterBlock* c, uint32_t nparts, uint32_t* occ_gate, hipStream_t s);
int shade_sections(unsigned long long* out, int n, int reset);

void launch_emitter_weights(const DevScene& sc, const float4* emis, float* weight, uint32_t* id, hipStream_t s);

constexpr int kOccRecF4 = 4;
void launch_occ_records(const DevScene& sc, uint32_t nnodes, float4* rec, hipStream_t s);
void launch_occ_probes(const DevScene& sc, float4* ro, float4* rd, uint32_t nkeys, hipStream_t s);
void launch_occ_complete(const DevScene& sc, const mcpt::OccTree& tree, uint32_t nkeys, uint32_t* ndone, hipStream_t s);
void launch_cull_margins(float4* nodes, uint32_t npairs, const float4* tri, uint32_t ntri, float* tri_w,
                         uint32_t* pmax, int passes, bool plane, hipStream_t s);
// ... 146 lines not shown
```

### mc-path-tracer_amd/csrc/runtime.cpp

```cpp
#include <chrono>
#include <cstdio>

#include "runtime_internal.hpp"

extern "C" {

const char* mcpt_last_error(const mcpt_ctx* c) { return c ? c->err.c_str() : mcpt_host::global_error(); }

int mcpt_create(int device, const mcpt_config* cfg, mcpt_ctx** out) {
    if (!out) return set_err(nullptr, MCPT_E_INVALID, "out is null");
    *out = nullptr;
    int n = 0;
    if (hipGetDeviceCount(&n) != hipSuccess || n <= 0)
        return set_err(nullptr, MCPT_E_NODEVICE, "no HIP device visible (the backend has no CPU fallback)");
    if (device < 0 || device >= n) return set_err(nullptr, MCPT_E_INVALID, "device index out of range");
    hipDeviceProp_t prop;
    if (hipGetDeviceProperties(&prop, device) != hipSuccess)
        return set_err(nullptr, MCPT_E_HIP, "hipGetDeviceProperties failed");
    if (strncmp(prop.gcnArchName, "gfx950", 6) != 0)
        return set_err(nullptr, MCPT_E_NODEVICE, std::string("device is ") + prop.gcnArchName + ", code objects are gfx950 only");
    mcpt_ctx* c = new mcpt_ctx();
    c->device = device;
    c->num_cu = prop.multiProcessorCount;
    snprintf(c->devname, sizeof(c->devname), "%s (%s, %d CUs)", prop.name, prop.gcnArchName, prop.multiProcessorCount);
    if (cfg) c->cfg = *cfg;
    else { c->cfg.seed = 0x5EED2026ull; c->cfg.spp = 16; c->cfg.max_depth = 5; c->cfg.rr_depth = 3; c->cfg.tile_w = 256; c->cfg.tile_h = 256; }
    if (c->cfg.max_depth < 1 || c->cfg.max_depth > 200 || c->cfg.spp < 0 || (uint32_t)c->cfg.spp > kMaxSpp - 256) {
        delete c;
        return set_err(nullptr, MCPT_E_INVALID, "bad config (max_depth 1..200, spp 0..2^19-256)");
    }
    if (hipSetDevice(device) != hipSuccess || hipStreamCreateWithFlags(&c->stream, hipStreamNonBlocking) != hipSuccess) {
        delete c;
        return set_err(nullptr, MCPT_E_HIP, "stream creation failed");
    }
    if (hipMalloc(&c->cnt, sizeof(CounterBlock)) != hipSuccess || hipHostMalloc(&c->cnt_host, sizeof(CounterBlock)) != hipSuccess) {
        delete c;
        return set_err(nullptr, MCPT_E_NOMEM, "counter allocation failed");
    }
    (void)hipMemset(c->cnt, 0, sizeof(CounterBlock));
    if (launch_geometry(device, c->geom) != 0) {
        mcpt_destroy(c);
        return set_err(nullptr, MCPT_E_HIP, "occupancy query failed");
    }
    c->trace_parts_default = c->geom.trace_parts;
    *out = c;
    return MCPT_OK;
}

void mcpt_destroy(mcpt_ctx* c) {
    if (!c) return;
    (void)hipSetDevice(c->device);
    if (c->stream) (void)hipStreamSynchronize(c->stream);
    c->scene.reset();
    free_list(c->film_bufs);
    free_list(c->tmp_bufs);
    if (c->cnt) (void)hipFree(c->cnt);
    if (c->cnt_host) (void)hipHostFree(c->cnt_host);
    if (c->tiles) (void)hipFree(c->tiles);
    if (c->step_tile) (void)hipFree(c->step_tile);
    if (c->step_tile_h) (void)hipHostFree(c->step_tile_h);
    if (c->ext_q) (void)hipFree(c->ext_q);
    if (c->any_q) (void)hipFree(c->any_q);
    if (c->mat_q) (void)hipFree(c->mat_q);
    if (c->any_ray) (void)hipFree(c->any_ray);
    for (auto e : c->events) (void)hipEventDestroy(e);
    if (c->stream) (void)hipStreamDestroy(c->stream);
    delete c;
}

int mcpt_device_name(mcpt_ctx* c, char* buf, int32_t len) {
    if (!c || !buf || len <= 0) return MCPT_E_INVALID;
    snprintf(buf, (size_t)len, "%s", c->devname);
    return MCPT_OK;
}

int mcpt_debug_ray_counts(const mcpt_ctx* c, uint64_t* out) {
    if (!c || !out) return MCPT_E_INVALID;
    const CounterBlock& t = c->totals;
    const bool ok = c->totals_ok;
    out[0] = ok ? t.tot_ext : 0;
    out[1] = ok ? t.tot_ext_q : 0;
    out[2] = ok ? t.tot_any : 0;
    out[3] = ok ? t.tot_any_q : 0;
    for (int k = 0; ok && k < kShards; k++) out[3] -= t.tot_emit[k];
    out[4] = ok ? t.tot_occ : 0;
    return MCPT_OK;
}
int mcpt_debug_primary_stats(const mcpt_ctx* c, double* out4) {
    if (!c || !out4) return MCPT_E_INVALID;
    out4[0] = c->prim.ok ? (double)c->prim.lists : 0.0;
    out4[1] = c->prim.ok ? (double)c->prim.over : 0.0;
    out4[2] = c->totals_ok ? (double)c->totals.tot_prim : 0.0;
    out4[3] = (double)c->prim.build_ms;
    return (int)std::min<uint64_t>(c->prim.builds, 0x7fffffffull);
}
int mcpt_debug_discard_stats(const mcpt_ctx* c, uint64_t* out4) {
    if (!c || !out4) return MCPT_E_INVALID;
    for (int k = 0; k < 4; k++) out4[k] = c->totals_ok ? c->totals.tot_skip[k] : 0;
    return MCPT_OK;
}
int mcpt_debug_occ_complete_stats(const mcpt_ctx* c, double* out4) {
    if (!c || !out4) return MCPT_E_INVALID;
    out4[0] = (double)c->scene.occ_done_keys;
    out4[1] = c->totals_ok ? (double)c->totals.tot_done[0] : 0.0;
    out4[2] = c->totals_ok ? (double)c->totals.tot_done[1] : 0.0;
    out4[3] = (double)c->scene.occ_done_ms;
    return MCPT_OK;
}
int mcpt_debug_occ_stats(const mcpt_ctx* c, uint64_t* resolved, int32_t* enabled) {
    if (!c) return MCPT_E_INVALID;
    if (resolved) *resolved = c->totals_ok ? c->totals.tot_occ : 0;
    if (enabled) *enabled = c->scene.dev.occ != nullptr;
    return MCPT_OK;
}

int mcpt_camera_set(mcpt_ctx* c, const mcpt_camera* cam) {
    if (!c || !cam) return set_err(c, MCPT_E_INVALID, "null argument");
    mcpt::CamView nc = c->cam;
    memcpy(nc.ivp, cam->inv_view_proj, sizeof(nc.ivp));
    memcpy(nc.iv, cam->inv_view, sizeof(nc.iv));
    nc.lens_radius = cam->lens_radius;
    nc.focal = cam->focal;
    if (c->has_cam && memcmp(&nc, &c->cam, sizeof(nc)) != 0) c->film_stale = true;
    c->cam = nc;
    c->has_cam = true;
    return MCPT_OK;
}

int mcpt_set_material_emission(mcpt_ctx* c, int32_t nmat, const float* rgb) {
    if (!c) return MCPT_E_INVALID;
    if (!c->scene.ok) return set_err(c, MCPT_E_INVALID, "no scene uploaded");
    Emission& em = c->em;
    const size_t n = 3 * (size_t)c->scene.nmat;
    std::vector<float> now(n, 0.f);
    if (rgb) {
        if (nmat != c->scene.nmat) return set_err(c, MCPT_E_INVALID, "nmat differs from the uploaded scene's");
        for (size_t i = 0; i < n; i++)
            if (!(rgb[i] >= 0.f) || !(rgb[i] <= 3.402823466e+38f))
                return set_err(c, MCPT_E_INVALID, "emission must be finite and >= 0");
        now.assign(rgb, rgb + n);
    }
    const std::vector<float> was = em.rgb.empty() ? std::vector<float>(n, 0.f) : em.rgb;
    const bool changed = n && memcmp(was.data(), now.data(), n * sizeof(float)) != 0;
    if (changed || (rgb && em.rgb.empty())) {
        std::vector<float4> t4(c->scene.nmat);
        int32_t lit = 0;
        for (int32_t m = 0; m < c->scene.nmat; m++) {
            t4[m] = make_float4(now[3 * m], now[3 * m + 1], now[3 * m + 2], 0.f);
            lit += now[3 * m] != 0.f || now[3 * m + 1] != 0.f || now[3 * m + 2] != 0.f;
        }
        HIPCHK(c, hipSetDevice(c->device));
        HIPCHK(c, hipStreamSynchronize(c->stream));
        if (!em.tab.ensure(t4.size())) {
            em.drop();
            return set_err(c, MCPT_E_NOMEM, "hipMalloc: emission table");
        }
        em.lit = 0;
        if (!t4.empty()) HIPCHK(c, hipMemcpy(em.tab, t4.data(), t4.size() * sizeof(float4), hipMemcpyHostToDevice));
        em.lit = lit;
    }
    if (rgb) em.rgb = now;
    else em.drop();
    if (changed) {
        c->film_stale = true;
        c->tp.ok = false;
        return emitter_table_refresh(c);
    }
    return MCPT_OK;
}

int mcpt_material_emission_read(mcpt_ctx* c, float* rgb, int32_t* nmat) {
    if (!c || !nmat) return set_err(c, MCPT_E_INVALID, "null argument");
    const Emission& em = c->em;
    *nmat = (int32_t)(em.rgb.size() / 3);
    if (em.rgb.empty()) return 0;
    if (rgb) memcpy(rgb, em.rgb.data(), em.rgb.size() * sizeof(float));
    return em.lit;
}

static int set_tiles_internal(mcpt_ctx* c, const std::vector<int2>& t);

// ... 386 lines not shown
    if (!t.ok) {
        if (n > t.cnt.size() || !t.stats) {
            (void)hipStreamSynchronize(c->stream);
            t.release();
            if (!t.cnt.ensure(n) || !t.list.ensure(n * kPrimLine) || !t.stats.ensure(4)) return fail();
        }
        PrimaryBuildArgs ba{};
        ba.scene = c->scene.dev;
        ba.cam = c->cam;
        ba.W = (int)W;
        ba.H = (int)H;
        ba.cam_px = sa.cam_px;
        ba.cam_dir = sa.cam_dir;
        ba.cnt = t.cnt;
        ba.list = t.list;
        ba.stats = t.stats;
        hipEvent_t e0 = nullptr, e1 = nullptr;
        uint32_t st[2] = {0, 0};
        float ms = 0.f;
        const bool ok = hipEventCreate(&e0) == hipSuccess && hipEventCreate(&e1) == hipSuccess &&
                        hipMemsetAsync(t.stats, 0, 16, c->stream) == hipSuccess &&
                        hipEventRecord(e0, c->stream) == hipSuccess &&
                        (launch_primary_build(ba, c->stream), hipGetLastError() == hipSuccess) &&
                        hipEventRecord(e1, c->stream) == hipSuccess &&
                        hipMemcpyAsync(st, t.stats, sizeof(st), hipMemcpyDeviceToHost, c->stream) == hipSuccess &&
                        hipStreamSynchronize(c->stream) == hipSuccess && hipEventElapsedTime(&ms, e0, e1) == hipSuccess;
        if (e0) (void)hipEventDestroy(e0);
        if (e1) (void)hipEventDestroy(e1);
        if (!ok) return fail();
        t.ok = true;
        t.builds++;
        t.lists = st[0];
        t.over = st[1];
        t.build_ms = ms;
    }
    if (qn > t.q.size()) {
        (void)hipStreamSynchronize(c->stream);
        if (!t.q.ensure(qn)) return fail();
    }
    sa.prim_cnt = t.cnt;
    sa.prim_list = t.list;
    sa.prim_q = t.q;
}

extern "C++" int check_ready(mcpt_ctx* c) {
    if (!c) return MCPT_E_INVALID;
    if (!c->scene.ok) return set_err(c, MCPT_E_INVALID, "no scene uploaded");
    if (!c->has_cam) return set_err(c, MCPT_E_INVALID, "no camera set");
    if (!c->P) return set_err(c, MCPT_E_INVALID, "film not allocated");
    if (!c->ext_q || !c->any_q || !c->mat_q || !c->any_ray)
        return set_err(c, MCPT_E_NOMEM, "ray queues not allocated");
    return MCPT_OK;
}

static int enqueue_iteration(mcpt_ctx* c, size_t evbase, bool timing, const int2* tiles, int ntiles, const int* tile_base) {
    ShadeArgs sa;
    sa.scene = c->scene.dev;
    sa.cam = c->cam;
    sa.p = c->p;
    sa.tiles = tiles;
    sa.ntiles = ntiles;
    sa.tile_w = (int)c->tile_w;
    sa.tile_h = (int)c->tile_h;
    sa.W = (int)c->W;
    sa.H = (int)c->H;
    sa.spp = c->cfg.spp;
    sa.max_depth = c->cfg.max_depth;
    sa.rr_depth = c->cfg.rr_depth;
    sa.seed = c->cfg.seed;
    sa.slots = (int)c->slots;
    sa.slots_rcp = 1.0f / (float)c->slots;
    sa.npx = (uint32_t)c->npx;
    sa.compact = c->compact ? 1 : 0;
    sa.tile_base = tile_base;
    sa.ext_q = c->ext_q;
    sa.any_q = c->any_q;
    sa.mat_rec = reinterpret_cast<uint4*>(c->mat_q);
    sa.mat_beta = reinterpret_cast<float4*>(c->mat_q) + (size_t)kShards * c->ext_cap;
    sa.ext_cap = c->ext_cap;
    sa.any_cap = c->any_cap;
    sa.cnt = c->cnt;
    sa.blk_done = c->blk_done_off ? nullptr : c->blk_done;
    sa.skip = c->skip_discarded ? 1 : 0;
    sa.budget = c->ad.budget_on ? c->ad.budget.get() : nullptr;
    sa.emis = c->em.dev_table();
    const bool samp = c->es.active() && sa.emis && c->es.nee2.get() && c->es.vis.get();
    sa.emit_cdf = samp ? c->es.cdf.get() : nullptr;
    sa.emit_ent = samp ? c->es.ent.get() : nullptr;
    sa.emit_n = samp ? (int)c->es.tab.cdf.size() : 0;
    sa.emit_vis0 = samp ? (uint32_t)(2 * c->es.paths) : 0u;
    sa.nee2 = samp ? c->es.nee2.get() : nullptr;
    if (samp) sa.p.vis = c->es.vis;
    if (int rc = cam_table(c, c->W, c->H, &sa.cam_px, &sa.cam_dir)) return rc;
    prim_table(c, sa);
    const int bpt = shade_blocks_per_tile((int)(c->tile_w * c->tile_h), (int)c->slots);
    if (timing) HIPCHK(c, hipEventRecord(ev(c, evbase + 0), c->stream));
    if (sa.ntiles > 0)
        launch_shade(sa, sa.ntiles * bpt, c->geom, (c->cfg.flags & MCPT_FLAG_FIXED) != 0, c->stream);
    if (timing) HIPCHK(c, hipEventRecord(ev(c, evbase + 1), c->stream));
    if (sa.ntiles > 0) launch_primary(sa, c->geom, c->stream);
    TraceArgs ta{};
    ta.scene = c->scene.dev;
    ta.nshards = kShards;
    TraceSet& e = ta.set[0];
    e.ro = c->p.ray_o;
    e.rd = c->p.ray_d;
    e.queue = c->ext_q;
    e.count_ptr = &c->cnt->shard[0][C_EXT];
    e.shard_cap = c->ext_cap;
    e.stats = c->count_work ? &c->cnt->shard[0][C_STATS] : nullptr;
    e.prefiltered = 1;
    TraceSet& v = ta.set[1];
    v.ro = c->p.sray_o;
    v.rd = c->p.sray_d;
    v.queue = c->any_q;
    v.count_ptr = &c->cnt->shard[0][C_ANY];
    v.shard_cap = c->any_cap;
    v.stats = c->count_work ? &c->cnt->shard[0][C_STATS + 3] : nullptr;
    v.prefiltered = 1;
    v.ray_at_slot = 1;
    ta.phase = c->count_work ? &c->cnt->shard[0][C_PH] : nullptr;
    ta.hit_tri = c->p.hit_tri;
    ta.vis = sa.p.vis;
    ta.grab = &c->cnt->grab[0][0];
    ta.idle = &c->cnt->idle;
    ta.tiny_stack = c->tiny_stack ? 1 : 0;
    launch_trace(ta, c->geom, c->stream);
    if (timing) HIPCHK(c, hipEventRecord(ev(c, evbase + 2), c->stream));
    launch_accumulate(c->cnt, c->geom.trace_parts, c->scene.dev.occ ? c->scene.dev.occ_gate : nullptr, c->stream);
    HIPCHK(c, hipGetLastError());
    return MCPT_OK;
}

static int run_iterations(mcpt_ctx* c, uint32_t n, mcpt_stage_stats* st, const int2* tiles = nullptr, int ntiles = -1,
                          const int* tile_base = nullptr) {
    int rc = check_ready(c);
    if (rc) return rc;
    HIPCHK(c, hipSetDevice(c->device));
    if (c->film_stale && !(c->cfg.flags & MCPT_FLAG_NO_AUTO_CLEAR) && (rc = mcpt_film_clear(c))) return rc;
    if (c->es.active()) {
        EmitterSampling& es = c->es;
        const size_t paths = c->npx * c->slots;
        if (es.paths != paths || !es.nee2.get() || !es.vis.get()) {
            if (3 * (uint64_t)paths >= (1ull << 32)) return set_err(c, MCPT_E_INVALID, "film too large for emitter sampling");
            HIPCHK(c, hipStreamSynchronize(c->stream));
            es.drop_streams();
            if (!es.nee2.ensure(paths) || !es.vis.ensure(3 * paths)) {
                es.drop_streams();
                return set_err(c, MCPT_E_NOMEM, "hipMalloc: emitter sampling streams");
            }
            HIPCHK(c, hipMemset(es.nee2, 0, paths * sizeof(float4)));
            HIPCHK(c, hipMemset(es.vis, 0, 3 * paths));
            es.paths = paths;
        }
    }
    if (!tiles) {
        tiles = c->tiles;
        ntiles = (int)c->tiles_h.size();
    }
    if (!c->totals_ok) {
        HIPCHK(c, hipMemcpyAsync(c->cnt_host, c->cnt, sizeof(CounterBlock), hipMemcpyDeviceToHost, c->stream));
        HIPCHK(c, hipStreamSynchronize(c->stream));
        c->totals = *c->cnt_host;
        c->totals_ok = true;
    }
    const CounterBlock before = c->totals;
// ... 102 lines not shown
    if (st) *st = acc;
    if (acc.live_paths != 0) return set_err(c, MCPT_E_INVALID, "render did not converge within the iteration cap");
    return MCPT_OK;
}

int mcpt_sync(mcpt_ctx* c) {
    if (!c) return MCPT_E_INVALID;
    HIPCHK(c, hipSetDevice(c->device));
    HIPCHK(c, hipStreamSynchronize(c->stream));
    return MCPT_OK;
}

extern "C++" int film_view(mcpt_ctx* c, const float4** Ld, const uint32_t** samples) {
    if (c->slots <= 1 && !c->compact) {
        *Ld = c->p.Ld;
        *samples = c->p.samples;
        return MCPT_OK;
    }
    ResolveArgs a{c->p.Ld, c->p.samples, c->film_Ld, c->film_samples, (uint32_t)c->npx, (int)c->slots,
                  c->compact ? c->tiles : nullptr, (int)c->tile_w, (int)c->tile_h, (int)c->W, (int)c->H};
    launch_resolve(a, c->stream);
    HIPCHK(c, hipGetLastError());
    *Ld = c->film_Ld;
    *samples = c->film_samples;
    return MCPT_OK;
}

static void unpack_target(mcpt_ctx* c, float4** Ld, uint32_t** samples) {
    *Ld = c->compact ? c->film_Ld : c->p.Ld;
    *samples = c->compact ? c->film_samples : c->p.samples;
}

int mcpt_set_path_slots(mcpt_ctx* c, uint32_t slots) {
    if (!c || slots < 1 || slots > 256) return set_err(c, MCPT_E_INVALID, "path slots must be 1..256");
    if (slots == c->slots) return MCPT_OK;
    if (!c->P) {
        c->slots = slots;
        return MCPT_OK;
    }
    if ((uint64_t)c->npx * slots >= (1ull << 31)) return set_err(c, MCPT_E_INVALID, "film too large for the path slots");
    const uint32_t old = c->slots;
    c->slots = slots;
    if (c->compact) {
        HIPCHK(c, hipSetDevice(c->device));
        const std::vector<int2> t = c->tiles_h;
        const size_t P = c->P;
        c->P = 0;
        int rc = set_tiles_internal(c, t);
        if (!rc) rc = alloc_film_state(c);
        if (rc != MCPT_OK) {
            const std::string err = c->err;
            c->slots = old;
            if (set_tiles_internal(c, t) == MCPT_OK && alloc_film_state(c) == MCPT_OK) {
                c->P = P;
                (void)mcpt_film_clear(c);
            }
            return set_err(c, rc, err);
        }
        c->P = P;
        return mcpt_film_clear(c);
    }
    int rc = film_resize(c, c->W, c->H, c->tile_w, c->tile_h);
    if (rc != MCPT_OK) {
        const std::string err = c->err;
        c->slots = old;
        (void)film_resize(c, c->W, c->H, c->tile_w, c->tile_h);
        return set_err(c, rc, err);
    }
    return MCPT_OK;
}

int mcpt_set_work_counters(mcpt_ctx* c, int32_t on) {
    if (!c) return MCPT_E_INVALID;
    c->count_work = on != 0;
    return MCPT_OK;
}

int mcpt_set_skip_discarded(mcpt_ctx* c, int32_t on) {
    if (!c) return MCPT_E_INVALID;
    c->skip_discarded = on != 0;
    return MCPT_OK;
}

int mcpt_set_trace_partitions(mcpt_ctx* c, uint32_t nparts) {
    if (!c || nparts > (uint32_t)kMaxParts)
        return set_err(c, MCPT_E_INVALID, "trace partitions must be 0 (device default) .. " + std::to_string(kMaxParts));
    c->geom.trace_parts = nparts ? nparts : c->trace_parts_default;
    return MCPT_OK;
}

int mcpt_film_read(mcpt_ctx* c, float* Ld, uint32_t* samples) {
    if (!c || !c->P) return set_err(c, MCPT_E_INVALID, "film not allocated");
    HIPCHK(c, hipSetDevice(c->device));
    const float4* fL;
    const uint32_t* fs;
    int rc = film_view(c, &fL, &fs);
    if (rc) return rc;
    HIPCHK(c, hipStreamSynchronize(c->stream));
    if (Ld && (rc = read_plane(c, fL, c->P, Ld, nullptr))) return rc;
    if (samples) HIPCHK(c, hipMemcpy(samples, fs, c->P * sizeof(uint32_t), hipMemcpyDeviceToHost));
    return MCPT_OK;
}

int mcpt_film_read_device(mcpt_ctx* c, void* dLd, void* dsamples) {
    if (!c || !c->P) return set_err(c, MCPT_E_INVALID, "film not allocated");
    HIPCHK(c, hipSetDevice(c->device));
    const float4* fL;
    const uint32_t* fs;
    int rc = film_view(c, &fL, &fs);
    if (rc) return rc;
    if (dLd) HIPCHK(c, hipMemcpyAsync(dLd, fL, c->P * sizeof(float4), hipMemcpyDeviceToDevice, c->stream));
    if (dsamples) HIPCHK(c, hipMemcpyAsync(dsamples, fs, c->P * sizeof(uint32_t), hipMemcpyDeviceToDevice, c->stream));
    HIPCHK(c, hipStreamSynchronize(c->stream));
    return MCPT_OK;
}

int mcpt_film_pack_tiles(mcpt_ctx* c, void* d_out, uint32_t* npix) {
    if (!c || !c->P) return set_err(c, MCPT_E_INVALID, "film not allocated");
    uint32_t n = (uint32_t)(c->tiles_h.size() * c->tile_w * c->tile_h);
    if (npix) *npix = n;
    if (!d_out) return MCPT_OK;
    HIPCHK(c, hipSetDevice(c->device));
    const float4* fL;
    const uint32_t* fs;
    int rc = film_view(c, &fL, &fs);
    if (rc) return rc;
    PackArgs a{fL, fs, c->tiles, (int)c->tiles_h.size(), (int)c->tile_w, (int)c->tile_h, (int)c->W, (int)c->H, (float4*)d_out};
    if (n) launch_pack(a, c->stream);
    HIPCHK(c, hipGetLastError());
    HIPCHK(c, hipStreamSynchronize(c->stream));
    return MCPT_OK;
}

int mcpt_film_unpack_tiles(mcpt_ctx* c, const void* d_in, const uint32_t* xy, uint32_t n) {
    if (!c || !c->P) return set_err(c, MCPT_E_INVALID, "film not allocated");
    if (n == 0) return MCPT_OK;
    if (!d_in || !xy) return set_err(c, MCPT_E_INVALID, "null argument");
    const uint32_t nx = (c->W + c->tile_w - 1) / c->tile_w, ny = (c->H + c->tile_h - 1) / c->tile_h;
    std::vector<int2> t(n);
    for (uint32_t i = 0; i < n; i++) {
        if (xy[2 * i] >= nx || xy[2 * i + 1] >= ny) return set_err(c, MCPT_E_INVALID, "tile out of range");
        t[i] = make_int2((int)xy[2 * i], (int)xy[2 * i + 1]);
        if (has_tile(c->tiles_h, t[i]))
            return set_err(c, MCPT_E_INVALID, "unpack into one of the context's own tiles");
    }
    HIPCHK(c, hipSetDevice(c->device));
    int2* dt = nullptr;
    HIPCHK(c, hipMalloc(&dt, n * sizeof(int2)));
    hipError_t e = hipMemcpyAsync(dt, t.data(), n * sizeof(int2), hipMemcpyHostToDevice, c->stream);
    if (e == hipSuccess) {
        float4* tL;
        uint32_t* ts;
        unpack_target(c, &tL, &ts);
        UnpackArgs ua{(const float4*)d_in, dt, (int)n, (int)c->tile_w, (int)c->tile_h, (int)c->W, (int)c->H, tL, ts};
        launch_unpack(ua, c->stream);
        e = hipGetLastError();
    }
    if (e == hipSuccess) e = hipStreamSynchronize(c->stream);
    (void)hipFree(dt);
    if (e != hipSuccess) return set_err(c, MCPT_E_HIP, std::string("unpack: ") + hipGetErrorString(e));
    for (const int2& x : t)
        if (!has_tile(c->unpacked, x)) c->unpacked.push_back(x);
    return MCPT_OK;
}

int mcpt_gather(mcpt_ctx* const* ctxs, int32_t n, int32_t root) {
// ... 113 lines not shown
```

### mc-path-tracer_amd/csrc/runtime_internal.hpp

```cpp
#pragma once
#include <hip/hip_runtime.h>

#include <algorithm>
#include <cstdlib>
#include <cstring>
#include <string>
#include <vector>

#include "host/emitter_table.hpp"
#include "kernels.hpp"
#include "mcpt.h"

using namespace mcpt_dev;

namespace mcpt_host {
void set_global_error(const std::string& e);
const char* global_error();
}

template <class T>
class DevBuf {
    T* p_ = nullptr;
    size_t n_ = 0;

// ... 141 lines not shown
};

struct UploadKnobs {
    bool cull_off = false;
    bool plane = true;
    int width = 0;
    int layout = -1;
    int occ_g = 24, occ_b = 12;
    bool occ_complete = true, occ_prefill = true;
    bool env_guides = true;
};

inline void free_list(std::vector<void*>& v) {
    for (void* q : v)
        if (q) (void)hipFree(q);
    v.clear();
}

struct SceneState {
    std::vector<void*> bufs;
    DevScene dev{};
    bool ok = false;
    int32_t ntri = 0;
    int32_t nmat = 0;
    UploadKnobs knobs;
    bool gpu_upload = false;
    const float4* pair_nodes = nullptr;
    uint32_t pair_count = 0;
    int pair_root = 0, pair_depth = 0, ploc_rounds = 0;
    int node_layout = 0;
    bool pair_gpu_built = false;
    bool cull_ok = true, nest_ok = true;
    float4* bvh_nodes = nullptr;
    uint32_t* order = nullptr;
    float4 *desc_tri = nullptr, *desc_sh = nullptr;
    float4* quads = nullptr;
    uint32_t* quad_src = nullptr;
    uint32_t nquads = 0;
    size_t occ_entries_n = 0;
    uint32_t* occ_init = nullptr;
    uint64_t occ_done_keys = 0;
    float occ_done_ms = 0.f;
    float4* occ_rec = nullptr;
    float4* occ_dir = nullptr;
    bool env_device_built = false;
    bool env_guides = false;
    float build_ms = 0.f;
    float env_build_ms = 0.f;
    DevBuf<float> stage;
    DevBuf<float4> box;
    DevBuf<float> tri_w, out;
    float update_ms[8] = {};

    void reset() {
        free_list(bufs);
        *this = SceneState{};
    }
    template <class T>
    void release(T*& p) {
        auto it = std::find(bufs.begin(), bufs.end(), (const void*)p);
        if (it != bufs.end()) {
            (void)hipFree(*it);
            bufs.erase(it);
        }
        p = nullptr;
    }
};

struct mcpt_ctx {
    int device = 0;
    hipStream_t stream = nullptr;
    std::string err;
    mcpt_config cfg{};
    char devname[256] = {0};
    int num_cu = 0;
    LaunchGeom geom{};
    uint32_t trace_parts_default = 1;
    SceneState scene;
    Emission em;
    EmitterSampling es;
    bool has_scene_before = false;
    bool count_work = getenv("MCPT_WORK_COUNTERS") != nullptr;
    bool skip_discarded = true;
    mcpt::CamView cam{};
    bool has_cam = false;
    CamTable cam_tab;
    PrimTable prim;
    uint64_t scene_gen = 0;
    bool film_stale = false;
    uint32_t W = 0, H = 0, tile_w = 256, tile_h = 256;
    size_t P = 0;
    uint32_t slots = 1;
    bool compact = false;
    size_t npx = 0;
    float4* film_Ld = nullptr;
    uint32_t* film_samples = nullptr;
    std::vector<void*> film_bufs;
    uint8_t* blk_done = nullptr;
    size_t blk_done_n = 0;
    bool blk_done_off = getenv("MCPT_NO_BLOCK_DONE") != nullptr;
    DevPaths p{};
    uint32_t *ext_q = nullptr, *any_q = nullptr, *mat_q = nullptr;
    float4* any_ray = nullptr;
    uint32_t ext_cap = 0, any_cap = 0;
    size_t queue_alloc = 0;
    uint32_t any_mult = 2, any_alloc_mult = 0;
    CounterBlock* cnt = nullptr;
    CounterBlock* cnt_host = nullptr;
    CounterBlock totals{};
    bool totals_ok = false;
    int2* step_tile = nullptr;
    int2* step_tile_h = nullptr;
    int2* tiles = nullptr;
    std::vector<int2> tiles_h;
    std::vector<int2> unpacked;
    uint32_t tiles_cap = 0;
    std::vector<hipEvent_t> events;
    std::vector<void*> tmp_bufs;
    float last_stage_ms = 0.f;
    int gpu_bvh_builder = MCPT_GPU_BVH_PLOC;
    bool tiny_stack = false;
    unsigned long long phase_base[kPhaseWords] = {};
    Guides guides;
    Denoise dn;
    Adaptive ad;
    Temporal tp;
    VarianceFill vf;
    StageMs ms;

    ViewKey view() const { return ViewKey{scene_gen, cfg.seed, W, H, cam}; }
};

inline int set_err(mcpt_ctx* c, int rc, const std::string& msg) {
    if (c) c->err = msg;
    mcpt_host::set_global_error(msg);
    return rc;
}
#define HIPCHK(c, x)                                                                          \
    do {                                                                                      \
        hipError_t e_ = (x);                                                                  \
        if (e_ != hipSuccess)                                                                 \
            return set_err((c), MCPT_E_HIP, std::string(#x) + ": " + hipGetErrorString(e_));  \
    } while (0)

template <class T>
int dalloc(mcpt_ctx* c, std::vector<void*>& list, T** out, size_t count) {
    void* q = nullptr;
    size_t bytes = std::max<size_t>(count * sizeof(T), 16);
    hipError_t e = hipMalloc(&q, bytes);
    if (e != hipSuccess) return set_err(c, MCPT_E_NOMEM, std::string("hipMalloc: ") + hipGetErrorString(e));
    list.push_back(q);
    *out = (T*)q;
    return MCPT_OK;
}
template <class T>
int dupload(mcpt_ctx* c, std::vector<void*>& list, T** out, const T* src, size_t count) {
    int rc = dalloc(c, list, out, count);
    if (rc) return rc;
    if (count) HIPCHK(c, hipMemcpy(*out, src, count * sizeof(T), hipMemcpyHostToDevice));
    return MCPT_OK;
}
struct TmpScope {
    std::vector<void*>& L;
    explicit TmpScope(mcpt_ctx* c) : L(c->tmp_bufs) { free_list(L); }
    ~TmpScope() { free_list(L); }
    TmpScope(const TmpScope&) = delete;
// ... 11 lines not shown
```

### mc-path-tracer_amd/mcpt/__init__.py

```python
from __future__ import annotations

import ctypes as C
import os
from dataclasses import dataclass

import numpy as np

_HERE = os.path.dirname(os.path.abspath(__file__))
PKG_DIR = os.path.dirname(_HERE)
REPO_DIR = os.path.dirname(PKG_DIR)
LIB_PATH = os.environ.get("MCPT_LIB") or os.path.join(PKG_DIR, "libmcpt.so")
ASSET_DIR = os.path.join(REPO_DIR, "assets")

MCPT_OK = 0
STAGE_LOGIC, STAGE_GENERATE, STAGE_MATERIAL, STAGE_EXTEND, STAGE_SHADOW = range(5)

_f = C.POINTER(C.c_float)
_i = C.POINTER(C.c_int32)
_u = C.POINTER(C.c_uint32)


class Config(C.Structure):
    _fields_ = [("seed", C.c_uint64), ("spp", C.c_int32), ("max_depth", C.c_int32), ("rr_depth", C.c_int32),
                ("tile_w", C.c_int32), ("tile_h", C.c_int32), ("flags", C.c_int32)]
# ... 102 lines not shown
    "mcpt_scene_upload": (C.c_int, [C.c_void_p, C.POINTER(SceneDesc)]),
    "mcpt_camera_set": (C.c_int, [C.c_void_p, C.POINTER(Camera)]),
    "mcpt_film_resize": (C.c_int, [C.c_void_p, C.c_uint32, C.c_uint32, C.c_uint32, C.c_uint32]),
    "mcpt_film_clear": (C.c_int, [C.c_void_p]),
    "mcpt_set_tiles": (C.c_int, [C.c_void_p, _u, C.c_uint32]),
    "mcpt_set_compact_paths": (C.c_int, [C.c_void_p, C.c_int32]),
    "mcpt_debug_tiny_lds_stack": (C.c_int, [C.c_void_p, C.c_int32]),
    "mcpt_set_path_slots": (C.c_int, [C.c_void_p, C.c_uint32]),
    "mcpt_set_trace_partitions": (C.c_int, [C.c_void_p, C.c_uint32]),
    "mcpt_gather": (C.c_int, [C.POINTER(C.c_void_p), C.c_int32, C.c_int32]),
    "mcpt_wavefront_step": (C.c_int, [C.c_void_p, C.c_uint32, C.c_uint32, C.POINTER(StageStats)]),
    "mcpt_iterate": (C.c_int, [C.c_void_p, C.c_uint32, C.POINTER(StageStats)]),
    "mcpt_render": (C.c_int, [C.c_void_p, C.POINTER(StageStats)]),
    "mcpt_stage_run": (C.c_int, [C.c_void_p, C.c_int, C.POINTER(SoaView), C.POINTER(SoaView), C.c_uint32]),
    "mcpt_film_read": (C.c_int, [C.c_void_p, _f, _u]),
    "mcpt_film_read_device": (C.c_int, [C.c_void_p, C.c_void_p, C.c_void_p]),
    "mcpt_film_pack_tiles": (C.c_int, [C.c_void_p, C.c_void_p, _u]),
    "mcpt_film_unpack_tiles": (C.c_int, [C.c_void_p, C.c_void_p, _u, C.c_uint32]),
    "mcpt_film_tonemap_rgba8": (C.c_int, [C.c_void_p, C.c_float, C.POINTER(C.c_uint8)]),
    "mcpt_guides_render": (C.c_int, [C.c_void_p, C.c_uint32]),
    "mcpt_guides_read": (C.c_int, [C.c_void_p, _f, _f, _f, _u]),
    "mcpt_denoise_default_params": (C.c_int, [C.POINTER(DenoiseParams)]),
    "mcpt_denoise_run": (C.c_int, [C.c_void_p, C.c_uint32, C.c_uint32, _f, _u, _f, _f, _f, C.POINTER(DenoiseParams), _f]),
    "mcpt_film_denoise": (C.c_int, [C.c_void_p, C.POINTER(DenoiseParams)]),
    "mcpt_denoised_read": (C.c_int, [C.c_void_p, _f]),
    "mcpt_denoised_read_device": (C.c_int, [C.c_void_p, C.c_void_p]),
    "mcpt_denoised_tonemap_rgba8": (C.c_int, [C.c_void_p, C.c_float, C.POINTER(C.c_uint8)]),
    "mcpt_denoised_write_png": (C.c_int, [C.c_void_p, C.c_float, C.c_char_p]),
    "mcpt_debug_denoise_ms": (C.c_int, [C.c_void_p, _f]),
    "mcpt_denoise_guided_default_params": (C.c_int, [C.POINTER(DenoiseGuidedParams)]),
    "mcpt_denoise_guided_run": (C.c_int, [C.c_void_p, C.c_uint32, C.c_uint32, _f, _u, _f, _f, _f, _f,
                                          C.POINTER(DenoiseGuidedParams), _f, _f]),
    "mcpt_film_denoise_guided": (C.c_int, [C.c_void_p, C.POINTER(DenoiseGuidedParams)]),
    "mcpt_denoised_variance_read": (C.c_int, [C.c_void_p, _f]),
    "mcpt_set_sample_budget": (C.c_int, [C.c_void_p, _u]),
    "mcpt_sample_budget_read": (C.c_int, [C.c_void_p, _u]),
    "mcpt_set_spp": (C.c_int, [C.c_void_p, C.c_int32]),
    "mcpt_film_error": (C.c_int, [C.c_void_p]),
    "mcpt_film_error_read": (C.c_int, [C.c_void_p, _f]),
    "mcpt_error_run": (C.c_int, [C.c_void_p, C.c_uint32, C.c_uint32, C.c_uint32, _f, _u, _f]),
    "mcpt_debug_film_read_slot": (C.c_int, [C.c_void_p, C.c_uint32, _f, _u]),
    "mcpt_sample_budget_default_params": (C.c_int, [C.POINTER(SampleBudgetParams)]),
    "mcpt_budget_from_error": (C.c_int, [C.c_void_p, C.POINTER(SampleBudgetParams), C.POINTER(C.c_uint64)]),
    "mcpt_debug_adaptive_bytes": (C.c_int64, [C.c_void_p]),
    "mcpt_debug_adaptive_ms": (C.c_int, [C.c_void_p, _f]),
    "mcpt_set_seed": (C.c_int, [C.c_void_p, C.c_uint64]),
    "mcpt_camera_view_proj": (C.c_int, [C.POINTER(Camera), _f]),
    "mcpt_temporal_default_params": (C.c_int, [C.POINTER(TemporalParams)]),
    "mcpt_film_temporal": (C.c_int, [C.c_void_p, C.POINTER(TemporalParams)]),
    "mcpt_temporal_reset": (C.c_int, [C.c_void_p]),
    "mcpt_temporal_read": (C.c_int, [C.c_void_p, _f, _f, _f, _f]),
    "mcpt_temporal_denoise": (C.c_int, [C.c_void_p, C.POINTER(DenoiseGuidedParams)]),
    "mcpt_temporal_run": (C.c_int, [C.c_void_p, C.c_uint32, C.c_uint32, _f, _u, _f, _f, _f, _f, _f, _f, _f, _f,
                                    C.POINTER(TemporalParams), _f, _f, _f, _f, _f]),
    "mcpt_debug_temporal_bytes": (C.c_int64, [C.c_void_p]),
    "mcpt_debug_temporal_ms": (C.c_int, [C.c_void_p, _f]),
    "mcpt_variance_default_params": (C.c_int, [C.POINTER(VarianceParams)]),
    "mcpt_variance_run": (C.c_int, [C.c_void_p, C.c_uint32, C.c_uint32, _f, _u, _f, _f, _f, _f, C.POINTER(VarianceParams), _f]),
    "mcpt_set_variance_fill": (C.c_int, [C.c_void_p, C.POINTER(VarianceParams)]),
    "mcpt_debug_variance_ms": (C.c_int, [C.c_void_p, _f]),
    "mcpt_set_material_emission": (C.c_int, [C.c_void_p, C.c_int32, _f]),
    "mcpt_material_emission_read": (C.c_int, [C.c_void_p, _f, _i]),
    "mcpt_set_emitter_sampling": (C.c_int, [C.c_void_p, C.c_int32]),
    "mcpt_emitter_table_read": (C.c_int, [C.c_void_p, _f, _f, _u, _i]),
    "mcpt_debug_emitter_stats": (C.c_int, [C.c_void_p, C.POINTER(C.c_double)]),
    "mcpt_scene_set_material_emission": (C.c_int, [C.c_void_p, C.c_int32, _f]),
    "mcpt_scene_get_emission": (C.c_int, [C.c_void_p, C.POINTER(_f), _i]),
    "mcpt_sync": (C.c_int, [C.c_void_p]),
    "mcpt_device_name": (C.c_int, [C.c_void_p, C.c_char_p, C.c_int32]),
    "mcpt_debug_queue_rays": (C.c_int, [C.c_void_p, C.c_int, _f, _f, _u]),
    "mcpt_debug_last_stage_ms": (C.c_float, [C.c_void_p]),
    "mcpt_debug_last_build_ms": (C.c_float, [C.c_void_p]),
    "mcpt_debug_last_env_build_ms": (C.c_float, [C.c_void_p]),
    "mcpt_debug_env_tables": (C.c_int, [C.c_void_p, _f, _f, _f, _i]),
    "mcpt_debug_node_layout": (C.c_int, [C.c_void_p]),
    "mcpt_debug_bvh_read": (C.c_int, [C.c_void_p, _f, _f, C.POINTER(BvhInfo)]),
    "mcpt_debug_occ_stats": (C.c_int, [C.c_void_p, C.POINTER(C.c_uint64), C.POINTER(C.c_int32)]),
    "mcpt_debug_occ_complete_stats": (C.c_int, [C.c_void_p, C.POINTER(C.c_double)]),
    "mcpt_debug_ray_counts": (C.c_int, [C.c_void_p, C.POINTER(C.c_uint64)]),
    "mcpt_debug_primary_stats": (C.c_int, [C.c_void_p, C.POINTER(C.c_double)]),
    "mcpt_set_work_counters": (C.c_int, [C.c_void_p, C.c_int32]),
    "mcpt_set_skip_discarded": (C.c_int, [C.c_void_p, C.c_int32]),
    "mcpt_debug_discard_stats": (C.c_int, [C.c_void_p, C.POINTER(C.c_uint64)]),
    "mcpt_scene_upload_gpu_bvh": (C.c_int, [C.c_void_p, C.c_void_p]),
    "mcpt_set_gpu_bvh_builder": (C.c_int, [C.c_void_p, C.c_int32]),
    "mcpt_scene_update_geometry": (C.c_int, [C.c_void_p, C.c_int32, _f, _f, _f, _f, _f, _f, C.c_int32]),
    "mcpt_scene_update_geometry_device": (C.c_int, [C.c_void_p, C.c_int32] + [C.c_void_p] * 6 + [C.c_int32]),
    "mcpt_debug_geometry_update_ms": (C.c_int, [C.c_void_p, _f]),
    "mcpt_film_size": (C.c_int, [C.c_void_p, C.POINTER(C.c_uint32), C.POINTER(C.c_uint32)]),
    "mcpt_film_write_png": (C.c_int, [C.c_void_p, C.c_float, C.c_char_p]),
    "mcpt_film_write_pfm": (C.c_int, [C.c_void_p, C.c_char_p]),
    "mcpt_image_write_png": (C.c_int, [C.c_char_p, C.c_uint32, C.c_uint32, C.POINTER(C.c_uint8)]),
    "mcpt_image_write_pfm": (C.c_int, [C.c_char_p, C.c_uint32, C.c_uint32, C.POINTER(C.c_float)]),
    "mcpt_debug_trace_profile": (C.c_int, [C.c_void_p, C.POINTER(C.c_uint64), C.c_int]),
    "mcpt_debug_shade_sections": (C.c_int, [C.c_void_p, C.POINTER(C.c_uint64), C.c_int, C.c_int]),
    "mcpt_scene_build_ex": (C.c_int, [C.c_void_p, C.c_void_p]),
    "mcpt_debug_quot": (C.c_int, [C.c_void_p, C.c_void_p, C.c_void_p, C.c_uint32, C.c_void_p]),
    "mcpt_debug_hbm_copy": (C.c_int, [C.c_void_p, C.c_uint64, C.c_uint32, C.POINTER(C.c_double)]),
    "mcpt_scene_new": (C.c_void_p, []),
    "mcpt_scene_free": (None, [C.c_void_p]),
    "mcpt_scene_load_glb": (C.c_int, [C.c_void_p, C.c_char_p, _f]),
    "mcpt_scene_add_mesh": (C.c_int, [C.c_void_p, C.c_int32, _f, _f, _f, _f, _f, _f, _f]),
    "mcpt_scene_set_env_hdr": (C.c_int, [C.c_void_p, C.c_char_p, C.c_int32]),
    "mcpt_scene_set_env_hdr_ex": (C.c_int, [C.c_void_p, C.c_char_p, C.c_int32, C.c_uint32]),
    "mcpt_scene_set_env_color": (C.c_int, [C.c_void_p, _f, C.c_float]),
    "mcpt_scene_add_dir_light": (C.c_int, [C.c_void_p, _f, _f, C.c_float]),
    "mcpt_scene_transform": (C.c_int, [C.c_void_p, _f]),
    "mcpt_scene_make_proxy": (C.c_int, [C.c_void_p, C.c_int32, C.c_char_p]),
    "mcpt_scene_build": (C.c_int, [C.c_void_p, C.c_int32]),
    "mcpt_scene_get_desc": (C.c_int, [C.c_void_p, C.POINTER(SceneDesc)]),
    "mcpt_scene_bvh_depth": (C.c_int, [C.c_void_p]),
    "mcpt_camera_make": (C.c_int, [C.POINTER(CameraParams), C.POINTER(Camera)]),
}

_lib = None


def lib() -> C.CDLL:
    global _lib
    if _lib is None:
        if not os.path.exists(LIB_PATH):
            raise RuntimeError(f"{LIB_PATH} missing: run __graft_entry__.build() (make) first")
        l = C.CDLL(LIB_PATH)
        for name, (res, args) in ABI.items():
            fn = getattr(l, name, None)
            if fn is None and os.environ.get("MCPT_LIB"):
                continue
            if fn is None:
                raise RuntimeError(f"{LIB_PATH} does not export {name}: rebuild it")
            fn.restype = res
            fn.argtypes = args
        _lib = l
    return _lib


class McptError(RuntimeError):
    pass


def _check(rc: int, ctx=None):
    if rc != MCPT_OK:
        msg = lib().mcpt_last_error(ctx)
        raise McptError(f"mcpt error {rc}: {msg.decode() if msg else ''}")


def fptr(a: np.ndarray):
    return a.ctypes.data_as(_f)


class BvhParams(C.Structure):
    _fields_ = [("builder", C.c_int32), ("max_prims", C.c_int32), ("buckets", C.c_int32),
                ("trav_cost", C.c_float), ("isect_cost", C.c_float)]


BVH_REFERENCE, BVH_SAH3 = 0, 1
FLAG_FIXED = 1
FLAG_NO_AUTO_CLEAR = 2
ENV_DEVICE_TABLES = 1
GEOM_MODES = {"refit": 0, "rebuild": 1}


def default_config(spp=16, max_depth=5, rr_depth=3, seed=0x5EED2026, tile=256, fixed=False,
                   auto_clear=True) -> Config:
    flags = (FLAG_FIXED if fixed else 0) | (0 if auto_clear else FLAG_NO_AUTO_CLEAR)
    return Config(seed, spp, max_depth, rr_depth, tile, tile, flags)

# ... 212 lines not shown
        return cdf, pick, tid

    def emitter_stats(self):
        out = (C.c_double * 4)()
        rc = lib().mcpt_debug_emitter_stats(self.h, out)
        if rc < 0:
            self._ck(rc)
        return {"entries": int(out[0]), "total_weight": out[1], "emitter_rays": int(out[2]), "build_ms": out[3],
                "active": rc == 1}

    def emission(self):
        n = C.c_int32(0)
        rc = lib().mcpt_material_emission_read(self.h, None, C.byref(n))
        if rc < 0:
            self._ck(rc)
        if n.value == 0:
            return None
        e = np.zeros((n.value, 3), np.float32)
        rc = lib().mcpt_material_emission_read(self.h, fptr(e), C.byref(n))
        if rc < 0:
            self._ck(rc)
        return e

    def update_geometry(self, v0, v1, v2, n0=None, n1=None, n2=None, mode="refit"):
        if mode not in GEOM_MODES:
            raise ValueError(f"unknown geometry update mode {mode!r}")
        arrs = [v0, v1, v2, n0, n1, n2]
        if all(hasattr(a, "data_ptr") for a in arrs if a is not None) and v0 is not None:
            import torch

            keep = []
            for a in arrs:
                if a is not None:
                    if not a.is_cuda or a.dtype != torch.float32:
                        raise ValueError("device arrays must be float32 tensors on the GPU")
                    if a.device.index != self.device:
                        raise ValueError(f"device arrays must be on the context's GPU {self.device}, not {a.device}")
                    a = a.contiguous()
                keep.append(a)
            n = keep[0].numel() // 3
            if any(a is not None and a.numel() != 3 * n for a in keep):
                raise ValueError("vertex arrays differ in size")
            torch.cuda.synchronize(keep[0].device)
            ptrs = [C.c_void_p(a.data_ptr()) if a is not None and a.numel() else None for a in keep]
            self._ck(lib().mcpt_scene_update_geometry_device(self.h, n, *ptrs, GEOM_MODES[mode]))
            return
        keep = [None if a is None else np.ascontiguousarray(a, np.float32).reshape(-1, 3) for a in arrs]
        n = len(keep[0])
        if any(a is not None and len(a) != n for a in keep):
            raise ValueError("vertex arrays differ in size")
        self._ck(lib().mcpt_scene_update_geometry(self.h, n, *[None if a is None else fptr(a) for a in keep],
                                                  GEOM_MODES[mode]))

    def geometry_update_ms(self) -> dict:
        v = (C.c_float * 8)()
        self._ck(lib().mcpt_debug_geometry_update_ms(self.h, v))
        return dict(zip(("records", "tree", "quads", "occ_records", "prefill", "complete_keys", "total"), [float(x) for x in v[:7]]))

    def ray_counts(self) -> dict:
        v = (C.c_uint64 * 5)()
        if hasattr(lib(), "mcpt_debug_ray_counts") or not os.environ.get("MCPT_LIB"):
            self._ck(lib().mcpt_debug_ray_counts(self.h, v))
        return dict(zip(("extension", "extension_traversed", "any_hit", "any_hit_traversed", "any_hit_occluder_cache"),
                        [int(x) for x in v]))

    def primary_stats(self) -> dict:
        v = (C.c_double * 4)()
        n = lib().mcpt_debug_primary_stats(self.h, v)
        if n < 0:
            raise McptError(f"mcpt_debug_primary_stats failed ({n})")
        return dict(lists=int(v[0]), overflow=int(v[1]), resolved=int(v[2]), build_ms=float(v[3]), builds=int(n))

    def set_skip_discarded(self, on=True):
        if hasattr(lib(), "mcpt_set_skip_discarded") or not os.environ.get("MCPT_LIB"):
            self._ck(lib().mcpt_set_skip_discarded(self.h, int(bool(on))))

    def discard_stats(self) -> dict:
        v = (C.c_uint64 * 4)()
        if hasattr(lib(), "mcpt_debug_discard_stats") or not os.environ.get("MCPT_LIB"):
            self._ck(lib().mcpt_debug_discard_stats(self.h, v))
        return dict(zip(("extension_untraced", "any_hit_untraced", "evaluations_not_run", "doomed_in_place"),
                        [int(x) for x in v]))

    def occ_stats(self):
        r, e = C.c_uint64(0), C.c_int32(0)
        self._ck(lib().mcpt_debug_occ_stats(self.h, C.byref(r), C.byref(e)))
        return int(r.value), bool(e.value)

    def occ_complete_stats(self) -> dict:
        v = (C.c_double * 4)()
        if hasattr(lib(), "mcpt_debug_occ_complete_stats") or not os.environ.get("MCPT_LIB"):
            self._ck(lib().mcpt_debug_occ_complete_stats(self.h, v))
        return dict(keys=int(v[0]), unoccluded=int(v[1]), occluded=int(v[2]), build_ms=float(v[3]))

    @property
    def last_build_ms(self) -> float:
        return lib().mcpt_debug_last_build_ms(self.h)

    def bvh_read(self):
        bi = BvhInfo()
        self._ck(lib().mcpt_debug_bvh_read(self.h, None, None, C.byref(bi)))
        nodes = np.zeros((bi.npairs, 4, 4), np.float32)
        tris = np.zeros((bi.ntri, bi.tri_f4, 4), np.float32)
        self._ck(lib().mcpt_debug_bvh_read(self.h, fptr(nodes) if nodes.size else None,
                                           fptr(tris) if tris.size else None, C.byref(bi)))
        info = {k: getattr(bi, k) for k, _ in BvhInfo._fields_}
        for k in ("root_mn", "root_mx"):
            info[k] = np.array(list(info[k]), np.float32)
        info["cull_p"] = np.float32(info["cull_p"])
        return nodes, tris, info

    @property
    def last_env_build_ms(self) -> float:
        return lib().mcpt_debug_last_env_build_ms(self.h)

    def env_tables(self, W, H) -> dict:
        my = np.zeros(H, np.float32)
        cy = np.zeros((H, W), np.float32)
        pdf = np.zeros((H, W), np.float32)
        fl = C.c_int32(0)
        self._ck(lib().mcpt_debug_env_tables(self.h, fptr(my), fptr(cy), fptr(pdf), C.byref(fl)))
        return {"marginal_y": my, "conds_y": cy, "pdf": pdf, "device_built": bool(fl.value & 1),
                "guides": bool(fl.value & 2)}

    def set_camera(self, cam: Camera):
        self._ck(lib().mcpt_camera_set(self.h, C.byref(cam)))

    def resize(self, W, H, tile_w=256, tile_h=256):
        self._ck(lib().mcpt_film_resize(self.h, W, H, tile_w, tile_h))
        self.W, self.H, self.tile_w, self.tile_h = W, H, tile_w, tile_h

    def clear(self):
        self._ck(lib().mcpt_film_clear(self.h))

    def set_path_slots(self, slots):
        self._ck(lib().mcpt_set_path_slots(self.h, slots))

    def set_work_counters(self, on=True):
        if hasattr(lib(), "mcpt_set_work_counters") or not os.environ.get("MCPT_LIB"):
            self._ck(lib().mcpt_set_work_counters(self.h, int(bool(on))))

    def set_trace_partitions(self, nparts=0):
        self._ck(lib().mcpt_set_trace_partitions(self.h, nparts))

    def set_compact_paths(self, on=True):
        self._ck(lib().mcpt_set_compact_paths(self.h, int(bool(on))))

    def set_tiny_lds_stack(self, on=True):
        self._ck(lib().mcpt_debug_tiny_lds_stack(self.h, int(bool(on))))

    def set_tiles(self, tiles=None):
        if tiles is None:
            self._ck(lib().mcpt_set_tiles(self.h, None, 0))
        else:
            t = np.ascontiguousarray(tiles, np.uint32).reshape(-1, 2)
            self._ck(lib().mcpt_set_tiles(self.h, t.ctypes.data_as(_u), len(t)))

    def step(self, tile_x, tile_y) -> StageStats:
        st = StageStats()
        self._ck(lib().mcpt_wavefront_step(self.h, tile_x, tile_y, C.byref(st)))
        return st

    def iterate(self, n) -> StageStats:
        st = StageStats()
        self._ck(lib().mcpt_iterate(self.h, n, C.byref(st)))
        return st
# ... 428 lines not shown
```

Before: 11670.

## Resolve extension rays from occupancy-grid closest-hit lists inside shade

Adds an extension-key path to the shade kernel. When a bounce ray's occupancy cache entry is complete and the ray lies inside that cell's beam, the kernel tests the listed candidate triangles directly, writes hit_tri, and skips queuing the ray for full BVH traversal. An adaptive gate with exponential backoff turns the path off when few lookups resolve. The cost is extra shared memory per block (two more float4 slabs), additional register pressure and loads in shade, and new counters, in exchange for removing extension traces.

```diff
diff --git a/include/mcpt.h b/include/mcpt.h
--- a/include/mcpt.h
+++ b/include/mcpt.h
@@ -138,6 +138,7 @@
 int mcpt_set_trace_partitions(mcpt_ctx *ctx, uint32_t nparts);
 int mcpt_set_work_counters(mcpt_ctx *ctx, int32_t on);
 int mcpt_set_skip_discarded(mcpt_ctx *ctx, int32_t on);
+int mcpt_set_ext_keys(mcpt_ctx *ctx, int32_t on);
 int mcpt_set_tiles(mcpt_ctx *ctx, const uint32_t *tile_xy, uint32_t ntiles);
 int mcpt_set_compact_paths(mcpt_ctx *ctx, int32_t on);
 int mcpt_wavefront_step(mcpt_ctx *ctx, uint32_t tile_x, uint32_t tile_y, mcpt_stage_stats *st);
@@ -266,6 +267,8 @@
 int mcpt_debug_ray_counts(const mcpt_ctx *ctx, uint64_t *out);
 int mcpt_debug_primary_stats(const mcpt_ctx *ctx, double *out4);
 int mcpt_debug_discard_stats(const mcpt_ctx *ctx, uint64_t *out4);
+int mcpt_debug_ext_key_stats(const mcpt_ctx *ctx, uint64_t *out4);
+int mcpt_debug_path_hits(mcpt_ctx *ctx, int32_t *hit_tri, uint32_t *flags, uint64_t *n_inout);
 int mcpt_debug_trace_profile(mcpt_ctx *ctx, uint64_t *out12, int reset);
 int mcpt_debug_shade_sections(mcpt_ctx *ctx, uint64_t *out, int n, int reset);
 int mcpt_debug_quot(mcpt_ctx *ctx, const float *a, const float *b, uint32_t n, float *out);
diff --git a/include/mcpt.hpp b/include/mcpt.hpp
--- a/include/mcpt.hpp
+++ b/include/mcpt.hpp
@@ -469,6 +469,7 @@
     void set_path_slots(uint32_t slots) {
         detail::check(mcpt_set_path_slots(ctx_, slots), ctx_, "set_path_slots");
     }
+    void set_ext_keys(bool on) { detail::check(mcpt_set_ext_keys(ctx_, on ? 1 : 0), ctx_, "set_ext_keys"); }
     void set_display(bool on) { display_ = on; }
     const mcpt_stage_stats& last_stats() const { return stats_; }
     const mcpt_config& config() const { return cfg_; }
diff --git a/mc-path-tracer_amd/csrc/device/closest_list.hpp b/mc-path-tracer_amd/csrc/device/closest_list.hpp
--- /dev/null
+++ b/mc-path-tracer_amd/csrc/device/closest_list.hpp
@@ -0,0 +1,46 @@
+#pragma once
+#include "mcpt_core.hpp"
+
+namespace mcpt {
+
+MCPT_HD float ray_cull_iota(bool cull_ok, float cull_p, V3 d, V3 inv) {
+    const float inf = __builtin_huge_valf();
+    const float ax = __builtin_fabsf(inv.x), ay = __builtin_fabsf(inv.y), az = __builtin_fabsf(inv.z);
+    if (!(ax < inf && ay < inf && az < inf)) return -inf;
+    const float n2 = d.x * d.x + d.y * d.y + d.z * d.z;
+    if (!cull_ok || !(n2 <= kCullNormMax)) return -3.4028235e38f;
+    const float io = __builtin_fmaxf(__builtin_fmaxf(ax, ay), az) * kCullSlackF;
+    return io * cull_p <= 1.f ? io : -io;
+}
+MCPT_HD bool inv_finite(V3 inv) {
+    const float inf = __builtin_huge_valf();
+    return __builtin_fabsf(inv.x) < inf && __builtin_fabsf(inv.y) < inf && __builtin_fabsf(inv.z) < inf;
+}
+MCPT_HD bool list_ray_ok(bool cull_ok, float cull_p, V3 d, V3 inv) {
+    return inv_finite(inv) && ray_cull_iota(cull_ok, cull_p, d, inv) > 0.f;
+}
+
+MCPT_HD bool list_accept(V3 o, V3 d, V3 inv, float4 bmn, float4 bmx, float4 r2, float4 r3, float bound, float& t) {
+    const float ax = (bmn.x - o.x) * inv.x, bx = (bmx.x - o.x) * inv.x;
+    const float ay = (bmn.y - o.y) * inv.y, by = (bmx.y - o.y) * inv.y;
+    const float az = (bmn.z - o.z) * inv.z, bz = (bmx.z - o.z) * inv.z;
+    const float t0 = __builtin_fmaxf(__builtin_fmaxf(__builtin_fminf(ax, bx), __builtin_fminf(ay, by)),
+                                     __builtin_fminf(az, bz));
+    const float t1 = __builtin_fminf(__builtin_fminf(__builtin_fmaxf(ax, bx), __builtin_fmaxf(ay, by)),
+                                     __builtin_fmaxf(az, bz));
+    return t0 <= t1 && tri_test_t(o, d, v3(bmx.w, r2.x, r2.y), v3(r2.z, r2.w, r3.x), v3(r3.y, r3.z, r3.w), t) &&
+           !(t < 0.f) && t < bound;
+}
+
+template <class SceneId>
+MCPT_HD void list_take(V3 o, V3 d, V3 inv, float4 bmn, float4 bmx, float4 r2, float4 r3, uint32_t id, SceneId sid,
+                       float& best, int32_t& tri) {
+    float t;
+    if (!list_accept(o, d, inv, bmn, bmx, r2, r3, K_HUGE, t)) return;
+    if (t < best || (t == best && tri >= 0 && sid(id) < sid((uint32_t)tri))) {
+        best = t;
+        tri = (int32_t)id;
+    }
+}
+
+}
diff --git a/mc-path-tracer_amd/csrc/kernels.hip b/mc-path-tracer_amd/csrc/kernels.hip
--- a/mc-path-tracer_amd/csrc/kernels.hip
+++ b/mc-path-tracer_amd/csrc/kernels.hip
@@ -4,6 +4,7 @@
 #include <string.h>
 #include <algorithm>
 
+#include "device/closest_list.hpp"
 #include "device/mcpt_core.hpp"
 #include "device/scene_dev.hpp"
 #include "kernels.hpp"
@@ -171,12 +172,7 @@
 constexpr float K_INF_F = __builtin_huge_valf();
 
 __device__ inline float cull_iota(const DevScene& sc, V3 d, V3 inv) {
-    const float ax = __builtin_fabsf(inv.x), ay = __builtin_fabsf(inv.y), az = __builtin_fabsf(inv.z);
-    if (!(ax < K_INF_F && ay < K_INF_F && az < K_INF_F)) return -K_INF_F;
-    const float n2 = d.x * d.x + d.y * d.y + d.z * d.z;
-    if (!sc.cull_ok || !(n2 <= kCullNormMax)) return -3.4028235e38f;
-    const float io = __builtin_fmaxf(__builtin_fmaxf(ax, ay), az) * kCullSlackF;
-    return io * sc.cull_p <= 1.f ? io : -io;
+    return mcpt::ray_cull_iota(sc.cull_ok != 0, sc.cull_p, d, inv);
 }
 __device__ inline bool keep_box(float t0, float t1, float m, float cut, float& key) {
     key = t0 - __builtin_fabsf(m);
@@ -337,13 +333,34 @@
     return done && fin && io > 0.f ? kOccMaybe : kOccOpen;
 }
 __device__ inline void occ_member2(const DevScene& sc, V3 ol, V3 dl, uint32_t kl, V3 ob, V3 db, uint32_t kb, bool& m_l,
-                                   bool& m_b) {
+                                   bool& m_b, bool want_e, V3 oe, V3 de, uint32_t ke, bool& m_e) {
     const mcpt::OccGrid g{{sc.root_mn[0], sc.root_mn[1], sc.root_mn[2]}, {sc.occ_cell[0], sc.occ_cell[1], sc.occ_cell[2]},
                           sc.occ_g, sc.occ_b, sc.occ_dir};
+    if (!want_e) ke = 0u;
     const mcpt::Beam bl = mcpt::occ_key_beam(g, (kl >> 15) & 31u, (kl >> 20) & 31u, kl >> 25, kl & 0x7fffu);
     const mcpt::Beam bb = mcpt::occ_key_beam(g, (kb >> 15) & 31u, (kb >> 20) & 31u, kb >> 25, kb & 0x7fffu);
+    const mcpt::Beam be = mcpt::occ_key_beam(g, (ke >> 15) & 31u, (ke >> 20) & 31u, ke >> 25, ke & 0x7fffu);
     m_l = mcpt::beam_contains(bl, ol, dl);
     m_b = mcpt::beam_contains(bb, ob, db);
+    m_e = want_e && mcpt::beam_contains(be, oe, de);
+}
+__device__ inline int32_t ext_key_hit(const DevScene& sc, V3 o, V3 d, V3 inv, OccEnt e) {
+    float best = K_HUGE;
+    int32_t tri = -1;
+    const auto sid = [&](uint32_t r) { return __float_as_int(sc.tri[kTriF4 * (size_t)r + 2].y); };
+#pragma unroll
+    for (uint32_t k = 0; k < kOccWays; k += 2) {
+        const uint32_t i0 = e.w[k] & mcpt::kOccDoneIndex, i1 = e.w[k + 1] & mcpt::kOccDoneIndex;
+        const bool v0 = i0 < sc.ntri, v1 = i1 < sc.ntri;
+        if (kOccWays > 2 && !(v0 || v1)) continue;
+        const float4* p0 = sc.occ_rec + kOccRecF4 * (size_t)(v0 ? i0 : 0u);
+        const float4* p1 = sc.occ_rec + kOccRecF4 * (size_t)(v1 ? i1 : 0u);
+        const float4 bn0 = p0[0], bx0 = p0[1], r20 = p0[2], r30 = p0[3];
+        const float4 bn1 = p1[0], bx1 = p1[1], r21 = p1[2], r31 = p1[3];
+        if (v0) mcpt::list_take(o, d, inv, bn0, bx0, r20, r30, i0, sid, best, tri);
+        if (v1) mcpt::list_take(o, d, inv, bn1, bx1, r21, r31, i1, sid, best, tri);
+    }
+    return tri;
 }
 
 struct MatOut {
@@ -353,6 +370,8 @@
     uint32_t trivial_any;
     OccEnt el, eb;
     uint32_t kl, kb;
+    OccEnt ee;
+    bool try_e;
     V3 n, wo, wi_b;
     int matid, light_id;
     uint32_t flags;
@@ -361,11 +380,12 @@
 
 template <bool FIXED, bool SAMP = false>
 __device__ inline MatOut material(const ShadeArgs& a, uint32_t pid, uint32_t pix, uint32_t sidx, uint32_t len,
-                                 V3 beta_store, int32_t htri, float4* stage, bool occ_on, bool no_cont, bool& want_e) {
+                                 V3 beta_store, int32_t htri, float4* stage, bool occ_on, bool ext_on, bool no_cont,
+                                 bool& want_e) {
     const DevScene& sc = a.scene;
     MatOut mo{};
 #pragma unroll
-    for (uint32_t k = 0; k < kOccWays; k++) mo.el.w[k] = mo.eb.w[k] = kOccEmpty;
+    for (uint32_t k = 0; k < kOccWays; k++) mo.el.w[k] = mo.eb.w[k] = mo.ee.w[k] = kOccEmpty;
     MCPT_MARK("m_hit");
     const Rng r{rng_key(a.seed, pix, sidx), len};
     const V3 ro = xyz(ld_s(a.p.ray_o + pid)), rdir = xyz(ld_s(a.p.ray_d + pid));
@@ -411,6 +431,12 @@
                 mo.want_ext = false;
                 mo.trivial_ext = true;
                 mo.doomed_inplace = doomed;
+            } else if (ext_on) {
+                uint32_t ke;
+                mo.ee = occ_entry(sc, occ_index(sc, new_o, wi_s, &ke));
+                stage[(SAMP ? 6 : 4) * kBlock + threadIdx.x] = f4(new_o, __uint_as_float(ke));
+                stage[(SAMP ? 7 : 5) * kBlock + threadIdx.x] = f4(wi_s, 0.f);
+                mo.try_e = true;
             }
         }
     }
@@ -871,7 +897,10 @@
     uint32_t n_emit = 0;
     (void)n_emit;
     const bool occ_on = a.scene.occ && a.scene.occ_gate[0] == 0 && a.scene.occ_gate[2] != 0;
-    __shared__ float4 s_any[SAMP ? 6 : 4][kBlock];
+    const bool ext_on = occ_on && a.ext_keys && a.scene.occ_dir && a.scene.occ_gate[3] == 0;
+    uint32_t n_etry = 0, n_ehit = 0, n_emiss = 0;
+    __shared__ float4 s_any[SAMP ? 8 : 6][kBlock];
+    constexpr int kExtSlab = SAMP ? 6 : 4;
     for (uint32_t base = w_in * kBlock; base < n; base += bps * kBlock) {
         const ShadeArgs& a = kernarg_fresh<ShadeArgs>();
         const uint32_t i = base + threadIdx.x;
@@ -880,12 +909,13 @@
         uint32_t mpid = 0;
         bool occ_l = false, occ_b = false, try_l = false, try_b = false;
         bool done_l = false, done_b = false, clr_l = false, clr_b = false;
+        bool try_e = false, key_hit = false, key_miss = false;
         if (i < n) {
             const uint4 q = ld_s(a.mat_rec + shard * a.ext_cap + i);
             const float4 b4 = ld_s(a.mat_beta + shard * a.ext_cap + i);
             mpid = q.x;
             mo = material<FIXED, SAMP>(a, mpid, q.y, q.z & (kRecNoCont - 1u), q.z >> kRecLenShift, xyz(b4), (int32_t)q.w,
-                                 &s_any[0][0], occ_on, (q.z & kRecNoCont) != 0u, want_e);
+                                 &s_any[0][0], occ_on, ext_on, (q.z & kRecNoCont) != 0u, want_e);
             MCPT_MARK("m_occ");
             if (occ_on) {
                 try_l = mo.want_l;
@@ -902,11 +932,33 @@
                     occ_b = r == kOccHit;
                     clr_b = r == kOccMaybe;
                 }
-                if (clr_l || clr_b) {
+                V3 oe = v3(0.f, 0.f, 0.f), de = oe, inv_e = oe;
+                uint32_t ke = 0u;
+                bool need_e = false, m_e = false;
+                if (mo.try_e) {
+                    const float4 o4 = s_any[kExtSlab][threadIdx.x];
+                    oe = xyz(o4);
+                    de = xyz(s_any[kExtSlab + 1][threadIdx.x]);
+                    ke = __float_as_uint(o4.w);
+                    inv_e = v3(1.f / de.x, 1.f / de.y, 1.f / de.z);
+                    try_e = mcpt::inv_finite(inv_e);
+                    bool done_e = try_e;
+#pragma unroll
+                    for (uint32_t k = 0; k < kOccWays; k++) done_e = done_e && mcpt::occ_word_done(mo.ee.w[k]);
+                    need_e = done_e && mcpt::list_ray_ok(a.scene.cull_ok != 0, a.scene.cull_p, de, inv_e);
+                }
+                if (clr_l || clr_b || need_e) {
                     bool m_l, m_b;
-                    occ_member2(a.scene, ol, dl, mo.kl, ob, db, mo.kb, m_l, m_b);
+                    occ_member2(a.scene, ol, dl, mo.kl, ob, db, mo.kb, m_l, m_b, need_e, oe, de, ke, m_e);
                     clr_l = clr_l && m_l;
                     clr_b = clr_b && m_b;
+                }
+                if (m_e) {
+                    const int32_t tri = ext_key_hit(a.scene, oe, de, inv_e, mo.ee);
+                    a.p.hit_tri[mpid] = tri;
+                    mo.want_ext = false;
+                    key_hit = tri >= 0;
+                    key_miss = tri < 0;
                 }
                 if (clr_l) {
                     a.p.vis[2 * mpid] = 1;
@@ -983,7 +1035,10 @@
         occ_try += (uint32_t)(__popcll(__ballot(try_l)) + __popcll(__ballot(try_b)));
         n_dvis += (uint32_t)(__popcll(__ballot(clr_l)) + __popcll(__ballot(clr_b)));
         n_docc += (uint32_t)(__popcll(__ballot(occ_l && done_l)) + __popcll(__ballot(occ_b && done_b)));
-        n_ext += (uint32_t)__popcll(__ballot(mo.want_ext || mo.trivial_ext || mo.skip_ext));
+        n_ext += (uint32_t)__popcll(__ballot(mo.want_ext || mo.trivial_ext || mo.skip_ext || key_hit || key_miss));
+        n_etry += (uint32_t)__popcll(__ballot(try_e));
+        n_ehit += (uint32_t)__popcll(__ballot(key_hit));
+        n_emiss += (uint32_t)__popcll(__ballot(key_miss));
         n_skip += (uint32_t)__popcll(__ballot(mo.skip_ext));
         n_inpl += (uint32_t)__popcll(__ballot(mo.doomed_inplace));
         n_any += (uint32_t)(__popcll(__ballot(mo.want_l)) + __popcll(__ballot(mo.want_b)) +
@@ -1000,6 +1055,9 @@
         if (n_docc) atomicAdd(sc_ctr + C_OCC_DONE_OCC, n_docc);
         if (n_skip) atomicAdd(sc_ctr + C_SKIP_EXT, n_skip);
         if (n_inpl) atomicAdd(sc_ctr + C_SKIP_INPLACE, n_inpl);
+        if (n_etry) atomicAdd(sc_ctr + C_EXT_KEY_TRY, n_etry);
+        if (n_ehit) atomicAdd(sc_ctr + C_EXT_KEY_HIT, n_ehit);
+        if (n_emiss) atomicAdd(sc_ctr + C_EXT_KEY_MISS, n_emiss);
         if constexpr (SAMP)
             if (n_emit) atomicAdd(a.cnt->tot_emit + shard, (unsigned long long)n_emit);
     }
@@ -1584,16 +1642,8 @@
                 if (j0 + k >= nc) break;
                 const float4* p = rec + kOccRecF4 * (size_t)id4[k];
                 const float4 bmn = p[0], bmx = p[1], r2 = p[2], r3 = p[3];
-                const float ax = (bmn.x - o.x) * inv.x, bx = (bmx.x - o.x) * inv.x;
-                const float ay = (bmn.y - o.y) * inv.y, by = (bmx.y - o.y) * inv.y;
-                const float az = (bmn.z - o.z) * inv.z, bz = (bmx.z - o.z) * inv.z;
-                const float t0 = __builtin_fmaxf(__builtin_fmaxf(__builtin_fminf(ax, bx), __builtin_fminf(ay, by)),
-                                                 __builtin_fminf(az, bz));
-                const float t1 = __builtin_fminf(__builtin_fminf(__builtin_fmaxf(ax, bx), __builtin_fmaxf(ay, by)),
-                                                 __builtin_fmaxf(az, bz));
                 float t;
-                if (t0 <= t1 && tri_test_t(o, d, v3(bmx.w, r2.x, r2.y), v3(r2.z, r2.w, r3.x), v3(r3.y, r3.z, r3.w), t) &&
-                    !(t < 0.f) && t < best) {
+                if (list_accept(o, d, inv, bmn, bmx, r2, r3, best, t)) {
                     best = t;
                     tri = (int32_t)id4[k];
                 }
@@ -1649,6 +1699,14 @@
         sk[k] = c->shard[t][skw[k]];
         if (sk[k]) c->shard[t][skw[k]] = 0;
         for (int off = 32; off > 0; off >>= 1) sk[k] += __shfl_xor(sk[k], off);
+    }
+    const int ekw[3] = {C_EXT_KEY_TRY, C_EXT_KEY_HIT, C_EXT_KEY_MISS};
+    uint32_t ek[3];
+#pragma unroll
+    for (int k = 0; k < 3; k++) {
+        ek[k] = c->shard[t][ekw[k]];
+        if (ek[k]) c->shard[t][ekw[k]] = 0;
+        for (int off = 32; off > 0; off >>= 1) ek[k] += __shfl_xor(ek[k], off);
     }
     c->shard[t][C_PRIM] = 0;
     c->shard[t][C_PRIM_RAYS] = 0;
@@ -1689,9 +1747,21 @@
                     occ_gate[1] = 0;
                 }
             }
-        }
+            if (occ_gate[3]) {
+                occ_gate[3]--;
+                c->tot_ext_key[3] += 1;
+            } else if (ek[0] >= 4096u) {
+                if (((unsigned long long)ek[1] + ek[2]) * kOccMinRate < ek[0]) {
+                    occ_gate[4] = occ_gate[4] ? min(2u * occ_gate[4] + 1u, 255u) : (uint32_t)MCPT_OCC_BACKOFF0;
+                    occ_gate[3] = occ_gate[4];
+                } else {
+                    occ_gate[4] = 0;
+                }
+            }
+        }
+        for (int k = 0; k < 3; k++) c->tot_ext_key[k] += ek[k];
         c->tot_vis += v[C_VIS];
-        c->tot_ext_q += v[C_EXT];
+        c->tot_ext_q += v[C_EXT] + ek[1] + ek[2];
         c->tot_any_q += v[C_ANY];
         c->last_ext = v[C_EXT];
         c->last_live = er;
diff --git a/mc-path-tracer_amd/csrc/kernels.hpp b/mc-path-tracer_amd/csrc/kernels.hpp
--- a/mc-path-tracer_amd/csrc/kernels.hpp
+++ b/mc-path-tracer_amd/csrc/kernels.hpp
@@ -82,7 +82,7 @@
 #endif
 constexpr uint32_t kOccWays = MCPT_OCC_WAYS;
 static_assert(kOccWays == 2 || kOccWays == 4, "an entry is one 8-B or 16-B load");
-constexpr uint32_t kOccGateWords = 3;
+constexpr uint32_t kOccGateWords = 5;
 constexpr uint32_t kOccMinRate = 10;
 __host__ __device__ constexpr size_t occ_entries(int g, int b) { return (size_t)g * g * g * 6 * b * b * kOccWays; }
 
@@ -97,7 +97,8 @@
 constexpr int kMaxParts = kShards;
 enum : int { C_EXT = 0, C_ANY = 1, C_VIS = 2, C_STATS = 3, C_EXT_RAYS = 9, C_ANY_RAYS = 10, C_MAT = 11, C_OCC = 12,
               C_OCC_TRY = 13, C_PH = 14, C_SKIP_INPLACE = 25, C_PRIM = 26, C_PRIM_RAYS = 27, C_SKIP_EXT = 28,
-              C_SKIP_ANY = 29, C_SKIP_MAT = 30, C_OCC_DONE_VIS = 31, C_OCC_DONE_OCC = 32, C_WORDS = 64 };
+              C_SKIP_ANY = 29, C_SKIP_MAT = 30, C_OCC_DONE_VIS = 31, C_OCC_DONE_OCC = 32, C_EXT_KEY_TRY = 33,
+              C_EXT_KEY_HIT = 34, C_EXT_KEY_MISS = 35, C_WORDS = 64 };
 enum : int {
     PH_TRIPS = 0,
     PH_REFILLS = 1,
@@ -128,6 +129,7 @@
     unsigned long long tot_skip[4];
     unsigned long long tot_done[2];
     unsigned long long tot_emit[kShards];
+    unsigned long long tot_ext_key[4];
 };
 static_assert(C_PH + kPhaseWords <= C_SKIP_INPLACE, "counter words overlap");
 
@@ -161,6 +163,7 @@
     const uint32_t* prim_list;
     uint2* prim_q;
     int skip;
+    int ext_keys;
     const uint32_t* budget;
     const float4* emis;
     const float* emit_cdf;
diff --git a/mc-path-tracer_amd/csrc/runtime.cpp b/mc-path-tracer_amd/csrc/runtime.cpp
--- a/mc-path-tracer_amd/csrc/runtime.cpp
+++ b/mc-path-tracer_amd/csrc/runtime.cpp
@@ -97,6 +97,24 @@
 int mcpt_debug_discard_stats(const mcpt_ctx* c, uint64_t* out4) {
     if (!c || !out4) return MCPT_E_INVALID;
     for (int k = 0; k < 4; k++) out4[k] = c->totals_ok ? c->totals.tot_skip[k] : 0;
+    return MCPT_OK;
+}
+int mcpt_debug_ext_key_stats(const mcpt_ctx* c, uint64_t* out4) {
+    if (!c || !out4) return MCPT_E_INVALID;
+    for (int k = 0; k < 4; k++) out4[k] = c->totals_ok ? c->totals.tot_ext_key[k] : 0;
+    return MCPT_OK;
+}
+int mcpt_debug_path_hits(mcpt_ctx* c, int32_t* hit_tri, uint32_t* flags, uint64_t* n_inout) {
+    if (!c || !n_inout) return MCPT_E_INVALID;
+    const uint64_t P = (uint64_t)c->npx * c->slots;
+    const uint64_t room = *n_inout;
+    *n_inout = P;
+    if (!hit_tri && !flags) return MCPT_OK;
+    if (room < P || !c->p.hit_tri || !c->p.flags) return set_err(c, MCPT_E_INVALID, "path hits: no film, or a short buffer");
+    HIPCHK(c, hipSetDevice(c->device));
+    HIPCHK(c, hipStreamSynchronize(c->stream));
+    if (hit_tri) HIPCHK(c, hipMemcpy(hit_tri, c->p.hit_tri, P * sizeof(int32_t), hipMemcpyDeviceToHost));
+    if (flags) HIPCHK(c, hipMemcpy(flags, c->p.flags, P * sizeof(uint32_t), hipMemcpyDeviceToHost));
     return MCPT_OK;
 }
 int mcpt_debug_occ_complete_stats(const mcpt_ctx* c, double* out4) {
@@ -649,6 +667,7 @@
     sa.cnt = c->cnt;
     sa.blk_done = c->blk_done_off ? nullptr : c->blk_done;
     sa.skip = c->skip_discarded ? 1 : 0;
+    sa.ext_keys = c->ext_keys ? 1 : 0;
     sa.budget = c->ad.budget_on ? c->ad.budget.get() : nullptr;
     sa.emis = c->em.dev_table();
     const bool samp = c->es.active() && sa.emis && c->es.nee2.get() && c->es.vis.get();
@@ -917,6 +936,12 @@
     return MCPT_OK;
 }
 
+int mcpt_set_ext_keys(mcpt_ctx* c, int32_t on) {
+    if (!c) return MCPT_E_INVALID;
+    c->ext_keys = on != 0;
+    return MCPT_OK;
+}
+
 int mcpt_set_trace_partitions(mcpt_ctx* c, uint32_t nparts) {
     if (!c || nparts > (uint32_t)kMaxParts)
         return set_err(c, MCPT_E_INVALID, "trace partitions must be 0 (device default) .. " + std::to_string(kMaxParts));
diff --git a/mc-path-tracer_amd/csrc/runtime_internal.hpp b/mc-path-tracer_amd/csrc/runtime_internal.hpp
--- a/mc-path-tracer_amd/csrc/runtime_internal.hpp
+++ b/mc-path-tracer_amd/csrc/runtime_internal.hpp
@@ -247,6 +247,7 @@
     bool has_scene_before = false;
     bool count_work = getenv("MCPT_WORK_COUNTERS") != nullptr;
     bool skip_discarded = true;
+    bool ext_keys = true;
     mcpt::CamView cam{};
     bool has_cam = false;
     CamTable cam_tab;
diff --git a/mc-path-tracer_amd/mcpt/__init__.py b/mc-path-tracer_amd/mcpt/__init__.py
--- a/mc-path-tracer_amd/mcpt/__init__.py
+++ b/mc-path-tracer_amd/mcpt/__init__.py
@@ -208,6 +208,9 @@
     "mcpt_set_work_counters": (C.c_int, [C.c_void_p, C.c_int32]),
     "mcpt_set_skip_discarded": (C.c_int, [C.c_void_p, C.c_int32]),
     "mcpt_debug_discard_stats": (C.c_int, [C.c_void_p, C.POINTER(C.c_uint64)]),
+    "mcpt_set_ext_keys": (C.c_int, [C.c_void_p, C.c_int32]),
+    "mcpt_debug_ext_key_stats": (C.c_int, [C.c_void_p, C.POINTER(C.c_uint64)]),
+    "mcpt_debug_path_hits": (C.c_int, [C.c_void_p, C.c_void_p, C.c_void_p, C.POINTER(C.c_uint64)]),
     "mcpt_scene_upload_gpu_bvh": (C.c_int, [C.c_void_p, C.c_void_p]),
     "mcpt_set_gpu_bvh_builder": (C.c_int, [C.c_void_p, C.c_int32]),
     "mcpt_scene_update_geometry": (C.c_int, [C.c_void_p, C.c_int32, _f, _f, _f, _f, _f, _f, C.c_int32]),
@@ -586,6 +589,23 @@
         return dict(zip(("extension_untraced", "any_hit_untraced", "evaluations_not_run", "doomed_in_place"),
                         [int(x) for x in v]))
 
+    def set_ext_keys(self, on=True):
+        if hasattr(lib(), "mcpt_set_ext_keys") or not os.environ.get("MCPT_LIB"):
+            self._ck(lib().mcpt_set_ext_keys(self.h, int(bool(on))))
+
+    def ext_key_stats(self) -> dict:
+        v = (C.c_uint64 * 4)()
+        if hasattr(lib(), "mcpt_debug_ext_key_stats") or not os.environ.get("MCPT_LIB"):
+            self._ck(lib().mcpt_debug_ext_key_stats(self.h, v))
+        return dict(zip(("tried", "hit", "miss", "gated_iterations"), [int(x) for x in v]))
+
+    def path_hits(self):
+        n = C.c_uint64(0)
+        self._ck(lib().mcpt_debug_path_hits(self.h, None, None, C.byref(n)))
+        ht, fl = np.zeros(n.value, np.int32), np.zeros(n.value, np.uint32)
+        self._ck(lib().mcpt_debug_path_hits(self.h, ht.ctypes.data, fl.ctypes.data, C.byref(n)))
+        return ht, fl
+
     def occ_stats(self):
         r, e = C.c_uint64(0), C.c_int32(0)
         self._ck(lib().mcpt_debug_occ_stats(self.h, C.byref(r), C.byref(e)))
```

Result: no change. 11820 (median of 6 runs) (+1.4%).
